# shenyunhang/PPS

Hardware: NVIDIA B200
Metric: qxg_pairs_per_sec_distance_plus_rank (higher is better)
Workload: dtype f16x3-split fp32 (two scaled fp16 planes, fp32 accumulate)

## Files before the change

pps_b200/build.py:

```python
from __future__ import annotations

import os
import shutil
import subprocess

HERE = os.path.dirname(os.path.abspath(__file__))
CSRC = os.path.join(HERE, "csrc")
OUT_DIR = os.path.join(HERE, "_C")
LIB_PATH = os.path.join(OUT_DIR, "libpps_b200.so")
SOURCES = ["pps_pool.cu", "split_prep.cu", "dist_gemm.cu", "pairs.cu", "rank.cu", "triplet.cu", "rerank.cu", "c_api.cu", "pass.cu", "index.cu"]
HEADERS = [os.path.join(CSRC, "common.cuh"), os.path.join(CSRC, "ctx.cuh"), os.path.join(CSRC, "dist_tiles.cuh"), os.path.join(os.path.dirname(HERE), "include", "pps_b200.h")]

NVCC_FLAGS = [
    "-gencode", "arch=compute_100a,code=sm_100a",
    "-O3", "-lineinfo", "-std=c++17",
    "-Xcompiler", "-fPIC",
]
OBJ_DIR = os.path.join(OUT_DIR, "obj")


def nvcc_path():
    for cand in (os.environ.get("NVCC"), shutil.which("nvcc"), "/usr/local/cuda/bin/nvcc"):
        if cand and os.path.exists(cand):
            return cand
    return None


def is_stale() -> bool:
    if not os.path.exists(LIB_PATH):
        return True
    t = os.path.getmtime(LIB_PATH)
    deps = [os.path.join(CSRC, s) for s in SOURCES] + HEADERS
    return any(os.path.getmtime(d) > t for d in deps if os.path.exists(d))


def _compile_one(nvcc, src, obj, verbose):
    cmd = [nvcc] + NVCC_FLAGS + (["-Xptxas", "-v"] if verbose else []) + ["-c", "-o", obj, src]
    proc = subprocess.run(cmd, cwd=CSRC, stdout=subprocess.PIPE, stderr=subprocess.STDOUT, text=True)
    return src, proc.returncode, proc.stdout


def build(force: bool = False, verbose: bool = False) -> str:
    if not force and not is_stale():
        return LIB_PATH
    nvcc = nvcc_path()
    if nvcc is None:
        raise RuntimeError("nvcc not found: cannot build libpps_b200.so (set NVCC or install the CUDA toolkit)")
    os.makedirs(OBJ_DIR, exist_ok=True)
    hdr_t = max(os.path.getmtime(h) for h in HEADERS if os.path.exists(h))
    jobs, objs = [], []
    for src in SOURCES:
        obj = os.path.join(OBJ_DIR, os.path.splitext(src)[0] + ".o")
        objs.append(obj)
        src_t = max(os.path.getmtime(os.path.join(CSRC, src)), hdr_t)
        if force or not os.path.exists(obj) or os.path.getmtime(obj) < src_t:
            jobs.append((src, obj))
    log = []
    if jobs:
        from concurrent.futures import ThreadPoolExecutor
        with ThreadPoolExecutor(max_workers=min(len(jobs), os.cpu_count() or 1)) as pool:
            for src, rc, out in pool.map(lambda j: _compile_one(nvcc, j[0], j[1], verbose), jobs):
                log.append("== %s ==\n%s" % (src, out))
                if rc != 0:
                    raise RuntimeError("nvcc failed on %s (%d):\n%s" % (src, rc, out))
    tmp = LIB_PATH + ".tmp.%d" % os.getpid()
    cmd = [nvcc, "-gencode", "arch=compute_100a,code=sm_100a", "-shared", "-o", tmp] + objs
    proc = subprocess.run(cmd, cwd=CSRC, stdout=subprocess.PIPE, stderr=subprocess.STDOUT, text=True)
    if proc.returncode != 0:
        if os.path.exists(tmp):
            os.remove(tmp)
        raise RuntimeError("nvcc link failed (%d):\n%s" % (proc.returncode, proc.stdout))
    os.replace(tmp, LIB_PATH)
    if verbose:
        print("\n".join(log))
    return LIB_PATH


TEST_HOOKS_PATH = os.path.join(OUT_DIR, "libpps_b200_testhooks.so")


def build_test_hooks(force: bool = False) -> str:
    src = os.path.join(CSRC, "test_hooks.cu")
    deps = [src] + [h for h in HEADERS if os.path.exists(h)]
    if (not force and os.path.exists(TEST_HOOKS_PATH)
            and all(os.path.getmtime(d) <= os.path.getmtime(TEST_HOOKS_PATH) for d in deps)):
        return TEST_HOOKS_PATH
    nvcc = nvcc_path()
    if nvcc is None:
        raise RuntimeError("nvcc not found: cannot build the test hooks")
    os.makedirs(OUT_DIR, exist_ok=True)
    tmp = TEST_HOOKS_PATH + ".tmp.%d" % os.getpid()
    proc = subprocess.run([nvcc] + NVCC_FLAGS + ["-shared", "-o", tmp, "test_hooks.cu"], cwd=CSRC, stdout=subprocess.PIPE,
                          stderr=subprocess.STDOUT, text=True)
    if proc.returncode != 0:
        raise RuntimeError("nvcc failed on test_hooks.cu:\n%s" % proc.stdout)
    os.replace(tmp, TEST_HOOKS_PATH)
    return TEST_HOOKS_PATH


if __name__ == "__main__":
    print(build(force=True, verbose=True))
```

pps_b200/csrc/c_api.cu:

```cuda
#include "common.cuh"

#include <algorithm>
#include <atomic>
#include <cstdio>
#include <cstring>
#include <new>
#include <numeric>
#include <string>
#include <vector>

namespace pps {

static std::atomic<unsigned long long> g_launches{0};
static thread_local std::string g_cuda_err;

void note_launch() { g_launches.fetch_add(1, std::memory_order_relaxed); }

int cuda_fail(cudaError_t e, const char* what) {
  g_cuda_err = std::string(what ? what : "?") + ": " + cudaGetErrorName(e) + " (" + cudaGetErrorString(e) + ")";
  return PPS_ERR_CUDA;
}

int sm_count() {
  static thread_local int cached_dev = -1, cached = 148;
// ... 26 lines not shown

using namespace pps;

extern "C" int pps_abi_version(void) { return PPS_ABI_VERSION; }

extern "C" const char* pps_strerror(int code) {
  switch (code) {
    case PPS_OK: return "ok";
    case PPS_ERR_INVALID_ARG: return "invalid argument (null pointer, negative size or unknown enum)";
    case PPS_ERR_SHAPE: return "shape check failed";
    case PPS_ERR_ALIGN: return "pointer or leading dimension not aligned";
    case PPS_ERR_CUDA: return "CUDA call failed";
    case PPS_ERR_UNSUPPORTED: return "request not supported by this build";
    case PPS_ERR_WORKSPACE: return "workspace too small";
    case PPS_ERR_NO_VALID_QUERY: return "No valid query";
    case PPS_ERR_PASS_RESIZE: return "a speculative size bound of the pass was too small: repeat it with PPS_PASS_SIZING";
    case PPS_ERR_TOPK_OVERFLOW: return "top-k candidate buffer overflow: repeat the pass with PPS_PASS_NO_EPILOGUE_TOPK";
    default: return "unknown error code";
  }
}

extern "C" const char* pps_last_cuda_error(void) { return g_cuda_err.c_str(); }

extern "C" unsigned long long pps_kernel_launch_count(void) { return g_launches.load(std::memory_order_relaxed); }

extern "C" long long pps_pairs_count(const int64_t* query_ids, long long nq, const int64_t* gallery_ids,
                                     long long ng) {
  if (nq < 0 || ng < 0 || ng > 0x7fffffffLL) return PPS_ERR_INVALID_ARG;
  if (nq == 0 || ng == 0) return 0;
  if (!query_ids || !gallery_ids) return PPS_ERR_INVALID_ARG;
  std::vector<int64_t> sorted(gallery_ids, gallery_ids + ng);
  std::sort(sorted.begin(), sorted.end());
  long long total = 0;
  for (long long i = 0; i < nq; ++i) {
    auto r = std::equal_range(sorted.begin(), sorted.end(), query_ids[i]);
    total += (long long)(r.second - r.first);
  }
  return total;
}

extern "C" int pps_pairs_fill(const int64_t* query_ids, const int64_t* query_cams, long long nq,
                              const int64_t* gallery_ids, const int64_t* gallery_cams, long long ng,
                              int32_t* pair_off, int32_t* pair_q, int32_t* pair_g, uint8_t* pair_pos) {
  if (nq < 0 || ng < 0 || ng > 0x7fffffffLL || nq > 0x7fffffffLL) return PPS_ERR_INVALID_ARG;
  if (!pair_off) return PPS_ERR_INVALID_ARG;
  pair_off[0] = 0;
  if (nq == 0) return PPS_OK;
  if (!query_ids || !query_cams || (ng > 0 && (!gallery_ids || !gallery_cams))) return PPS_ERR_INVALID_ARG;
  IdIndex idx(gallery_ids, ng);
  long long e = 0;
  for (long long i = 0; i < nq; ++i) {
    size_t lo, hi;
    idx.range(query_ids[i], &lo, &hi);
    if (e + (long long)(hi - lo) > 0x7fffffffLL) return PPS_ERR_UNSUPPORTED;
    for (size_t s = lo; s < hi; ++s, ++e) {
      const int32_t g = idx.order[s];
      if (!pair_q || !pair_g || !pair_pos) return PPS_ERR_INVALID_ARG;
      pair_q[e] = (int32_t)i;
      pair_g[e] = g;
      pair_pos[e] = gallery_cams[g] != query_cams[i] ? 1 : 0;
    }
    pair_off[i + 1] = (int32_t)e;
  }
  return PPS_OK;
}

#include "ctx.cuh"

namespace {
inline void mark(pps_ctx* c, int i, cudaStream_t s) {
  if (c->timing && c->ev_phase[i]) cudaEventRecord(c->ev_phase[i], s);
}
}

extern "C" int pps_ctx_create(int device, pps_ctx** out) {
  if (!out) return PPS_ERR_INVALID_ARG;
  *out = nullptr;
  PPS_CUDA_TRY(cudaSetDevice(device));
  pps_ctx* c = new (std::nothrow) pps_ctx();
  if (!c) return PPS_ERR_INVALID_ARG;
  c->device = device;
  cudaError_t e = cudaStreamCreateWithFlags(&c->copy_s, cudaStreamNonBlocking);
  if (e == cudaSuccess) e = cudaStreamCreateWithFlags(&c->comp_s, cudaStreamNonBlocking);
  if (e == cudaSuccess) e = cudaStreamCreateWithFlags(&c->side_s, cudaStreamNonBlocking);
  if (e == cudaSuccess) e = cudaEventCreateWithFlags(&c->ev_in, cudaEventDisableTiming);
  if (e == cudaSuccess) e = cudaEventCreateWithFlags(&c->ev_pairs, cudaEventDisableTiming);
  for (int i = 0; i < kMaxSlabs && e == cudaSuccess; ++i) e = cudaEventCreateWithFlags(&c->ev_slab[i], cudaEventDisableTiming);
  if (e == cudaSuccess) e = cudaEventCreateWithFlags(&c->ev_totals, cudaEventDisableTiming);
  for (int i = 0; i <= PPS_N_PHASES && e == cudaSuccess; ++i) e = cudaEventCreate(&c->ev_phase[i]);
  if (e != cudaSuccess) {
    pps_ctx_destroy(c);
    return cuda_fail(e, "pps_ctx_create");
  }
  *out = c;
  return PPS_OK;
}

extern "C" int pps_ctx_destroy(pps_ctx* c) {
  if (!c) return PPS_OK;
  cudaSetDevice(c->device);
  if (c->comp_s) cudaStreamSynchronize(c->comp_s);
  if (c->copy_s) cudaStreamSynchronize(c->copy_s);
  if (c->side_s) cudaStreamSynchronize(c->side_s);
  GrowBuf* bufs[] = {&c->qf, &c->gf, &c->qs, &c->gs, &c->qn, &c->gn, &c->dist, &c->ids, &c->pair_ws, &c->pair_off,
                     &c->totals, &c->pair_q, &c->pair_pos, &c->xbuf, &c->counters, &c->ap,
                     &c->valid, &c->first, &c->topk, &c->tki, &c->tkd};
  for (GrowBuf* b : bufs) b->release();
  c->h_small.release();
  c->pass.release();
  for (int i = 0; i < kMaxSlabs; ++i) if (c->ev_slab[i]) cudaEventDestroy(c->ev_slab[i]);
  if (c->ev_totals) cudaEventDestroy(c->ev_totals);
  if (c->ev_in) cudaEventDestroy(c->ev_in);
  if (c->ev_pairs) cudaEventDestroy(c->ev_pairs);
  if (c->side_s) cudaStreamDestroy(c->side_s);
  for (int i = 0; i <= PPS_N_PHASES; ++i) if (c->ev_phase[i]) cudaEventDestroy(c->ev_phase[i]);
  if (c->copy_s) cudaStreamDestroy(c->copy_s);
  if (c->comp_s) cudaStreamDestroy(c->comp_s);
  delete c;
  return PPS_OK;
}

namespace {

int eval_shape(long long nq, long long ng, long long col0, int dim, int precision, int topk, EvalShape* e) {
  if (nq <= 0 || ng <= 0 || dim <= 0 || topk < 0 || topk > PPS_TOPK_MAX || col0 < 0) return PPS_ERR_INVALID_ARG;
  if (nq > 0x7fffffffLL || col0 + ng > 0x7fffffffLL) return PPS_ERR_UNSUPPORTED;
  switch (precision) {
    case PPS_PREC_BF16X1: e->planes = 1; break;
    case PPS_PREC_BF16X3: e->planes = 2; break;
    case PPS_PREC_BF16X6: e->planes = 3; break;
    case PPS_PREC_F16X3: e->planes = 2; break;
    default: return PPS_ERR_INVALID_ARG;
  }
  e->split_planes = precision == PPS_PREC_F16X3 ? (2 | PPS_SPLIT_F16_SCALED) : e->planes;
  e->nq = nq; e->ng = ng; e->col0 = col0; e->dim = dim; e->precision = precision; e->topk = topk;
  e->ldd = (ng + 3) & ~3LL;
  e->kpad = pps_kpad(dim);
  if ((double)nq * (double)e->ldd * 4.0 > 64.0 * (double)(1LL << 30)) return PPS_ERR_UNSUPPORTED;
  return PPS_OK;
}

int ensure_common(pps_ctx* c, const EvalShape& e) {
  PPS_TRY(c->qs.ensure((size_t)pps_split_bytes(e.nq, e.dim, e.planes)));
  PPS_TRY(c->gs.ensure((size_t)pps_split_bytes(e.ng, e.dim, e.planes)));
  PPS_TRY(c->qn.ensure((size_t)e.nq * 8));
  PPS_TRY(c->gn.ensure((size_t)e.ng * 8));
  PPS_TRY(c->dist.ensure((size_t)e.nq * e.ldd * 4));
  PPS_TRY(c->pair_ws.ensure((size_t)pps_pairs_workspace_bytes(e.nq, e.ng)));
  PPS_TRY(c->pair_off.ensure(((size_t)e.nq + 1) * 4));
  PPS_TRY(c->totals.ensure(16));
  PPS_TRY(c->ap.ensure((size_t)e.nq * 8));
  PPS_TRY(c->valid.ensure((size_t)e.nq));
  PPS_TRY(c->first.ensure((size_t)e.nq * 4));
  const size_t off_ap = 16, off_first = off_ap + (size_t)e.nq * 8, off_valid = off_first + (size_t)e.nq * 4;
  PPS_TRY(c->h_small.ensure(off_valid + (size_t)e.nq));
  unsigned char* base = c->h_small.as<unsigned char>();
  c->st.totals = reinterpret_cast<int32_t*>(base);
  c->st.ap = reinterpret_cast<double*>(base + off_ap);
  c->st.first = reinterpret_cast<int32_t*>(base + off_first);
  c->st.valid = base + off_valid;
  return PPS_OK;
}

int pairs_local_count(pps_ctx* c, cudaStream_t ready_on) {
  const EvalShape& e = c->cur;
  cudaStream_t ps = c->pair_stream(ready_on);
  if (ready_on != ps) {
// ... 126 lines not shown

extern "C" int pps_evaluate_host_ctx(pps_ctx* c, const float* q_feats, long long nq, const float* g_feats, long long ng,
                                     int dim, const int64_t* query_ids, const int64_t* query_cams,
                                     const int64_t* gallery_ids, const int64_t* gallery_cams, int precision,
                                     int cmc_topk, int topk, double* out_map, double* out_cmc, double* out_ap,
                                     uint8_t* out_valid, int32_t* out_first_rank, int32_t* out_topk_index,
                                     float* out_topk_dist) {
  if (!c || cmc_topk < 0) return PPS_ERR_INVALID_ARG;
  PPS_TRY(eval_shape(nq, ng, 0, dim, precision, topk, &c->cur));
  c->world = 1;
  c->ext_pair_s = nullptr;
  const EvalShape& e = c->cur;
  if (!q_feats || !g_feats || !query_ids || !query_cams || !gallery_ids || !gallery_cams) return PPS_ERR_INVALID_ARG;
  if (!out_map || (cmc_topk > 0 && !out_cmc)) return PPS_ERR_INVALID_ARG;
  PPS_CUDA_TRY(cudaSetDevice(c->device));
  cudaStream_t cs = c->comp_s, ps = c->copy_s, ss = c->side_s;
  const int planes = e.planes, kpad = e.kpad;
  const long long ldd = e.ldd;

  PPS_TRY(ensure_common(c, e));
  PPS_TRY(c->qf.ensure((size_t)nq * dim * 4));
  PPS_TRY(c->gf.ensure((size_t)ng * dim * 4));
  PPS_TRY(c->ids.ensure((size_t)(2 * nq + 2 * ng) * 8));
  int64_t* d_qid = c->ids.as<int64_t>();
  int64_t* d_qcam = d_qid + nq;
  int64_t* d_gid = d_qcam + nq;
  int64_t* d_gcam = d_gid + ng;
  c->d_qid = d_qid; c->d_qcam = d_qcam; c->d_gid = d_gid; c->d_gcam = d_gcam;

  PPS_CUDA_TRY(cudaMemcpyAsync(d_qid, query_ids, (size_t)nq * 8, cudaMemcpyHostToDevice, ss));
  PPS_CUDA_TRY(cudaMemcpyAsync(d_qcam, query_cams, (size_t)nq * 8, cudaMemcpyHostToDevice, ss));
  PPS_CUDA_TRY(cudaMemcpyAsync(d_gid, gallery_ids, (size_t)ng * 8, cudaMemcpyHostToDevice, ss));
  PPS_CUDA_TRY(cudaMemcpyAsync(d_gcam, gallery_cams, (size_t)ng * 8, cudaMemcpyHostToDevice, ss));
  PPS_TRY(pairs_local_count(c, ss));
  PPS_TRY(pairs_offsets(c, c->local_cnt, 0, ss));

  PPS_CUDA_TRY(cudaMemcpyAsync(c->qf.p, q_feats, (size_t)nq * dim * 4, cudaMemcpyHostToDevice, cs));
  PPS_TRY(pps_split_rows(c->qf.p, PPS_DTYPE_F32, nq, dim, dim, e.split_planes, c->qs.p, c->qn.as<float>(), cs));

  long long slab = ((ng + 7) / 8 + 255) & ~255LL;
  if (slab < 1024) slab = 1024;
  while ((ng + slab - 1) / slab > kMaxSlabs) slab *= 2;
  int si = 0;
  const size_t esz = 2;
  for (long long r0 = 0; r0 < ng; r0 += slab, ++si) {
    const long long nr = std::min(slab, ng - r0);
    PPS_CUDA_TRY(cudaMemcpyAsync(c->gf.as<float>() + r0 * dim, g_feats + r0 * dim, (size_t)nr * dim * 4,
                                 cudaMemcpyHostToDevice, ps));
    PPS_CUDA_TRY(cudaEventRecord(c->ev_slab[si], ps));
    PPS_CUDA_TRY(cudaStreamWaitEvent(cs, c->ev_slab[si], 0));
    PPS_TRY(pps_split_rows_slab(c->gf.p, PPS_DTYPE_F32, r0, nr, ng, dim, dim, e.split_planes, c->gs.p, c->gn.as<float>(), cs));
    PPS_TRY(pps_dist_tc(c->qs.p, c->qn.as<float>(), nq, planes, 0,
                        c->gs.as<unsigned char>() + (size_t)r0 * kpad * esz, c->gn.as<float>() + r0, nr, planes, ng, dim,
                        precision, 0, c->dist.as<float>() + r0, ldd, cs));
  }
  int rc = pairs_and_thresholds(c, cs);
  if (rc == PPS_OK) rc = count_local(c, cs);
  if (rc == PPS_OK)
    rc = finalize_and_fetch(c, cmc_topk, cs, out_map, out_cmc, out_ap, out_valid, out_first_rank, out_topk_index,
                            out_topk_dist);
  cudaStreamSynchronize(ps);
  return rc;
}

extern "C" int pps_rank_begin(pps_ctx* c, const float* d_q, long long nq, const float* d_g, long long ng_local, int dim,
                              const int64_t* d_qid, const int64_t* d_qcam, const int64_t* d_gid_local,
                              const int64_t* d_gcam_local, long long gallery_offset, int world, int precision, int topk,
                              void* stream, void* pair_stream, int32_t** d_local_cnt) {
  if (!c || world < 1) return PPS_ERR_INVALID_ARG;
  PPS_TRY(eval_shape(nq, ng_local, gallery_offset, dim, precision, topk, &c->cur));
  if (!d_q || !d_g || !d_qid || !d_qcam || !d_gid_local || !d_gcam_local) return PPS_ERR_INVALID_ARG;
  PPS_CUDA_TRY(cudaSetDevice(c->device));
  cudaStream_t cs = static_cast<cudaStream_t>(stream);
  c->d_qid = d_qid; c->d_qcam = d_qcam; c->d_gid = d_gid_local; c->d_gcam = d_gcam_local;
  c->d_q = d_q; c->d_g = d_g;
  c->world = world;
  c->ext_pair_s = static_cast<cudaStream_t>(pair_stream);
  PPS_TRY(ensure_common(c, c->cur));
  const EvalShape& e = c->cur;
  mark(c, 0, cs);
  PPS_TRY(pairs_local_count(c, cs));
  if (d_local_cnt) *d_local_cnt = c->local_cnt;
  mark(c, 1, cs);
  PPS_TRY(pps_split_rows(d_q, PPS_DTYPE_F32, e.nq, e.dim, e.dim, e.split_planes, c->qs.p, c->qn.as<float>(), cs));
  PPS_TRY(pps_split_rows(d_g, PPS_DTYPE_F32, e.ng, e.dim, e.dim, e.split_planes, c->gs.p, c->gn.as<float>(), cs));
  mark(c, 2, cs);
  PPS_TRY(pps_dist_tc(c->qs.p, c->qn.as<float>(), e.nq, e.planes, 0, c->gs.p, c->gn.as<float>(), e.ng, e.planes, 0,
                      e.dim, e.precision, world > 1 ? PPS_DIST_RESERVE_SM_PAIR : 0, c->dist.as<float>(), e.ldd, cs));
  mark(c, 3, cs);
  return PPS_OK;
}

extern "C" int pps_rank_thresholds(pps_ctx* c, const int32_t* d_cnt_all, int rank, void* stream, long long* n_pairs,
                                   int32_t** d_exchange, long long* n_words) {
  if (!c || c->cur.nq <= 0 || rank < 0 || rank >= c->world) return PPS_ERR_INVALID_ARG;
  cudaStream_t cs = static_cast<cudaStream_t>(stream);
  PPS_TRY(pairs_offsets(c, d_cnt_all ? d_cnt_all : c->local_cnt, rank, cs));
  PPS_TRY(pairs_and_thresholds(c, cs));
  mark(c, 4, cs);
  if (n_pairs) *n_pairs = c->n_pairs;
  if (d_exchange) *d_exchange = c->xbuf.as<int32_t>();
  if (n_words) *n_words = 3 * c->n_pairs;
  return PPS_OK;
}

extern "C" int pps_rank_count_local(pps_ctx* c, void* stream, uint32_t** d_counters, long long* n_counters) {
  if (!c || c->cur.nq <= 0) return PPS_ERR_INVALID_ARG;
  cudaStream_t cs = static_cast<cudaStream_t>(stream);
  PPS_TRY(count_local(c, cs));
  mark(c, 5, cs);
  if (d_counters) *d_counters = c->counters.as<uint32_t>();
  if (n_counters) *n_counters = c->cur.nq + c->n_pairs;
  return PPS_OK;
}

extern "C" int pps_rank_end(pps_ctx* c, int cmc_topk, void* stream, double* out_map, double* out_cmc, double* out_ap,
                            uint8_t* out_valid, int32_t* out_first_rank, int32_t* out_topk_index,
                            float* out_topk_dist) {
  if (!c || c->cur.nq <= 0 || cmc_topk < 0) return PPS_ERR_INVALID_ARG;
  const int rc = finalize_and_fetch(c, cmc_topk, static_cast<cudaStream_t>(stream), out_map, out_cmc, out_ap, out_valid,
                                    out_first_rank, out_topk_index, out_topk_dist);
  if (rc == PPS_OK || rc == PPS_ERR_NO_VALID_QUERY) collect_phase_times(c);
  return rc;
}

extern "C" int pps_evaluate_device_ctx(pps_ctx* c, const float* d_q, long long nq, const float* d_g, long long ng,
                                       int dim, const int64_t* d_qid, const int64_t* d_qcam, const int64_t* d_gid,
                                       const int64_t* d_gcam, int precision, int cmc_topk, int topk, void* stream,
                                       double* out_map, double* out_cmc, double* out_ap, uint8_t* out_valid,
                                       int32_t* out_first_rank, int32_t* out_topk_index, float* out_topk_dist) {
  if (!out_map || (cmc_topk > 0 && !out_cmc)) return PPS_ERR_INVALID_ARG;
  PPS_TRY(pps_rank_begin(c, d_q, nq, d_g, ng, dim, d_qid, d_qcam, d_gid, d_gcam, 0, 1, precision, topk, stream, nullptr,
                         nullptr));
  PPS_TRY(pps_rank_thresholds(c, nullptr, 0, stream, nullptr, nullptr, nullptr));
  PPS_TRY(pps_rank_count_local(c, stream, nullptr, nullptr));
  return pps_rank_end(c, cmc_topk, stream, out_map, out_cmc, out_ap, out_valid, out_first_rank, out_topk_index,
                      out_topk_dist);
}

extern "C" int pps_ctx_set_timing(pps_ctx* c, int enabled) {
  if (!c) return PPS_ERR_INVALID_ARG;
  c->timing = enabled != 0;
  return PPS_OK;
}

extern "C" int pps_ctx_phase_ms(const pps_ctx* c, float* out_ms) {
  if (!c || !out_ms) return PPS_ERR_INVALID_ARG;
  for (int i = 0; i < PPS_N_PHASES; ++i) out_ms[i] = c->phase_ms[i];
  return PPS_OK;
}

extern "C" int pps_evaluate_host(const float* q_feats, long long nq, const float* g_feats, long long ng, int dim,
                                 const int64_t* query_ids, const int64_t* query_cams, const int64_t* gallery_ids,
                                 const int64_t* gallery_cams, int precision, int cmc_topk, int topk, int device,
                                 double* out_map, double* out_cmc, double* out_ap, uint8_t* out_valid,
                                 int32_t* out_first_rank, int32_t* out_topk_index, float* out_topk_dist) {
  pps_ctx* c = nullptr;
  int rc = pps_ctx_create(device, &c);
  if (rc != PPS_OK) return rc;
  rc = pps_evaluate_host_ctx(c, q_feats, nq, g_feats, ng, dim, query_ids, query_cams, gallery_ids, gallery_cams,
                             precision, cmc_topk, topk, out_map, out_cmc, out_ap, out_valid, out_first_rank,
                             out_topk_index, out_topk_dist);
  pps_ctx_destroy(c);
  return rc;
}
```

pps_b200/csrc/common.cuh:

```cuda
#pragma once

#include <cuda.h>
#include <cuda_runtime.h>
#include <cuda_bf16.h>
#include <cuda_fp16.h>
#include <stdint.h>

#include "../../include/pps_b200.h"

namespace pps {

void note_launch();
int  cuda_fail(cudaError_t e, const char* what);

#define PPS_CUDA_TRY(expr)                                            \
  do {                                                                \
    cudaError_t _e = (expr);                                          \
    if (_e != cudaSuccess) return ::pps::cuda_fail(_e, #expr);        \
  } while (0)

#define PPS_LAUNCH_CHECK(name)                                        \
  do {                                                                \
    ::pps::note_launch();                                             \
    cudaError_t _e = cudaGetLastError();                              \
    if (_e != cudaSuccess) return ::pps::cuda_fail(_e, name);         \
  } while (0)

int sm_count();

#ifdef __CUDACC__

__device__ __forceinline__ uint32_t smem_u32(const void* p) {
  return static_cast<uint32_t>(__cvta_generic_to_shared(p));
}

__device__ __forceinline__ void mbar_init(uint64_t* bar, uint32_t count) {
  asm volatile("mbarrier.init.shared::cta.b64 [%0], %1;" ::"r"(smem_u32(bar)), "r"(count) : "memory");
}
__device__ __forceinline__ void fence_barrier_init() {
  asm volatile("fence.mbarrier_init.release.cluster;" ::: "memory");
}
__device__ __forceinline__ void fence_proxy_async() {
  asm volatile("fence.proxy.async.shared::cta;" ::: "memory");
}
__device__ __forceinline__ void mbar_expect_tx(uint64_t* bar, uint32_t bytes) {
  asm volatile("mbarrier.arrive.expect_tx.shared::cta.b64 _, [%0], %1;" ::"r"(smem_u32(bar)), "r"(bytes)
               : "memory");
}
__device__ __forceinline__ void mbar_arrive(uint64_t* bar) {
  asm volatile("mbarrier.arrive.shared::cta.b64 _, [%0];" ::"r"(smem_u32(bar)) : "memory");
}
__device__ __forceinline__ bool mbar_try_wait(uint64_t* bar, uint32_t parity) {
  uint32_t ok;
  asm volatile(
      "{\n\t"
      ".reg .pred p;\n\t"
      "mbarrier.try_wait.parity.shared::cta.b64 p, [%1], %2;\n\t"
      "selp.u32 %0, 1, 0, p;\n\t"
      "}\n"
      : "=r"(ok)
      : "r"(smem_u32(bar)), "r"(parity)
      : "memory");
  return ok != 0;
}
__device__ __forceinline__ void mbar_wait(uint64_t* bar, uint32_t parity) {
  while (!mbar_try_wait(bar, parity)) {
  }
}

__device__ __forceinline__ void bulk_load_1d(void* smem_dst, const void* gsrc, uint32_t bytes, uint64_t* bar) {
  asm volatile(
      "cp.async.bulk.shared::cluster.global.mbarrier::complete_tx::bytes [%0], [%1], %2, [%3];" ::"r"(
          smem_u32(smem_dst)),
      "l"(gsrc), "r"(bytes), "r"(smem_u32(bar))
      : "memory");
}

__device__ __forceinline__ void tma_load_3d(void* smem_dst, const CUtensorMap* tmap, uint64_t* bar, int c0, int c1,
                                            int c2) {
  asm volatile(
      "cp.async.bulk.tensor.3d.shared::cluster.global.tile.mbarrier::complete_tx::bytes [%0], [%1, {%3, %4, %5}], "
      "[%2];" ::"r"(smem_u32(smem_dst)),
      "l"(reinterpret_cast<uint64_t>(tmap)), "r"(smem_u32(bar)), "r"(c0), "r"(c1), "r"(c2)
      : "memory");
}
__device__ __forceinline__ void tma_store_2d(const CUtensorMap* tmap, const void* smem_src, int c0, int c1) {
  asm volatile("cp.async.bulk.tensor.2d.global.shared::cta.tile.bulk_group [%0, {%2, %3}], [%1];" ::"l"(
                   reinterpret_cast<uint64_t>(tmap)),
               "r"(smem_u32(smem_src)), "r"(c0), "r"(c1)
               : "memory");
}
__device__ __forceinline__ void bulk_commit_group() { asm volatile("cp.async.bulk.commit_group;" ::: "memory"); }
template <int N>
__device__ __forceinline__ void bulk_wait_group_read() {
  asm volatile("cp.async.bulk.wait_group.read %0;" ::"n"(N) : "memory");
}
__device__ __forceinline__ float lds_f32(uint32_t addr) {
  float v;
  asm volatile("ld.shared.f32 %0, [%1];" : "=f"(v) : "r"(addr));
  return v;
}
__device__ __forceinline__ void red_shared_add_u32(uint32_t addr, uint32_t v) {
  asm volatile("red.shared.add.u32 [%0], %1;" ::"r"(addr), "r"(v) : "memory");
}
__device__ __forceinline__ uint32_t ld_volatile_u32(const uint32_t* p) {
  uint32_t v;
  asm volatile("ld.volatile.global.u32 %0, [%1];" : "=r"(v) : "l"(p) : "memory");
  return v;
}
__device__ __forceinline__ void st_volatile_u32(uint32_t* p, uint32_t v) {
  asm volatile("st.volatile.global.u32 [%0], %1;" ::"l"(p), "r"(v) : "memory");
// ... 148 lines not shown
```

pps_b200/csrc/ctx.cuh:

```cuda
#pragma once

#include "common.cuh"

#include <algorithm>
#include <cstring>
#include <new>
#include <vector>

namespace pps {

struct GrowBuf {
  void* p = nullptr;
  size_t cap = 0;
  int ensure(size_t bytes) {
    if (bytes <= cap) return PPS_OK;
    if (p) { cudaFree(p); p = nullptr; cap = 0; }
    const size_t want = bytes + bytes / 8 + 256;
    cudaError_t e = cudaMalloc(&p, want);
    if (e != cudaSuccess) { p = nullptr; return ::pps::cuda_fail(e, "cudaMalloc"); }
    cap = want;
    return PPS_OK;
  }
  void release() { if (p) cudaFree(p); p = nullptr; cap = 0; }
  template <class T> T* as() const { return static_cast<T*>(p); }
};

struct PinBuf {
  void* p = nullptr;
  size_t cap = 0;
  int ensure(size_t bytes) {
    if (bytes <= cap) return PPS_OK;
    if (p) { cudaFreeHost(p); p = nullptr; cap = 0; }
    cudaError_t e = cudaMallocHost(&p, bytes + 256);
    if (e != cudaSuccess) { p = nullptr; return ::pps::cuda_fail(e, "cudaMallocHost"); }
    cap = bytes + 256;
    return PPS_OK;
  }
  void release() { if (p) cudaFreeHost(p); p = nullptr; cap = 0; }
  template <class T> T* as() const { return static_cast<T*>(p); }
};

constexpr int kMaxSlabs = 64;

#define PPS_TRY(expr) do { int _rc = (expr); if (_rc != PPS_OK) return _rc; } while (0)

struct EvalShape {
  long long nq, ng , col0 , ldd;
  int dim, kpad, planes, precision, topk;
  int split_planes;
};
struct Staging {
  int32_t* totals; double* ap; int32_t* first; uint8_t* valid;
};

int pairs_count_device_ex(const int64_t* query_ids, long long nq, const int64_t* gallery_ids, long long ng_cap, void* workspace,
                          int32_t* pair_off, int32_t* totals, void* stream, const int32_t* ng_dev);
int pairs_fill_device_ex(const int64_t* query_ids, const int64_t* query_cams, long long nq, const int64_t* gallery_ids,
                         const int64_t* gallery_cams, long long ng_cap, const void* workspace, int32_t* pair_q, int32_t* pair_g,
                         uint8_t* pair_pos, float* zero_f32, uint32_t* zero_u32, uint32_t* zero_per_query, long long capacity,
                         void* stream, const int32_t* ng_dev);
int pairs_remap_ex(int32_t* pair_g, long long n_cap, const int32_t* cand_rows, long long offset, void* stream,
                   const int32_t* n_dev);
int pairs_compact_rows_ex(const int64_t* query_ids, long long nq, const int32_t* pair_off, const int32_t* pair_q,
                          const int32_t* pair_g, long long n_pairs, long long row_lo, long long row_hi, void* workspace,
                          int32_t* gp_rows, int32_t* pair_col, int32_t* n_rows, void* stream, const int32_t* n_pairs_dev,
                          long long rows_cap);
int rank_gather_ex(const float* dist, long long ldd, long long nq, long long ncols, long long col0, const int32_t* pair_q,
                   const int32_t* pair_g, long long n_pairs, float* pair_d, void* stream, const int32_t* n_dev);

constexpr int kPassMaxBlocks = 4096;
constexpr int kPassTimedLaunches = 256;
struct PassState {
  bool active = false;
  long long nq = 0, ngl = 0, ng_global = 0, offset = 0, chunk = 0, ldd = 0, n_pairs = 0, n_cand = 0, n_rows = 0;
  int dim = 0, kpad = 0, dtype = 0, planes = 0, split_planes = 0, precision = 0, topk = 0, world = 1, rank = 0, flags = 0;
  int max_pairs = 0, n_blocks = 0, tk_cap = 2048;
  bool prefilter = false, g_inplace = false, epi_topk = false;
  bool fused = false;
  int p_cap = 0;
  const void *d_q = nullptr, *d_g = nullptr;
  const void *h_q = nullptr, *h_g = nullptr;
  bool g_from_host = false;
  const int64_t *d_qid = nullptr, *d_qcam = nullptr, *d_gid = nullptr, *d_gcam = nullptr;
  long long blk_row0[kPassMaxBlocks], blk_rows[kPassMaxBlocks];
  size_t packed_bytes = 0;
  size_t res_bytes = 0, res_first_off = 0, res_valid_off = 0, res_flags_off = 0;
  GrowBuf qs, qn, gs, gn, dist, tdist, ts, tn, pair_ws, pair_off, totals, pair_q, pair_g, pair_pos, pair_d, packed, pf_ws,
      cand_rows, cand_gid, cand_gcam, gp_rows, pair_col, gp_ws, tk_bound, tk_cnt, tk_cand, small, ap, valid, first, tki, tkd,
      thr_tab, tpair_tab, cnt_tab, dstar, gstar;
  cudaEvent_t ev_a = nullptr, ev_rows = nullptr;
  cudaEvent_t ev_t[kPassTimedLaunches][2] = {};
  int n_timed = 0, timed_kind[kPassTimedLaunches] = {};
  float host_wait_ms[4] = {};
  struct Hints { bool valid = false; long long nq = 0, ng_global = 0, ngl = 0, offset = 0, mbb = 0; int dim = 0, dtype = 0, topk = 0,
                 world = 0, precision = 0; long long n_cand = 0, n_pairs = 0, n_rows = 0; int max_pairs = 0; } hints;
  bool speculative = false;
  long long cap_cand = 0, cap_rows = 0;
  void release() {
    GrowBuf* bufs[] = {&qs, &qn, &gs, &gn, &dist, &tdist, &ts, &tn, &pair_ws, &pair_off, &totals, &pair_q, &pair_g, &pair_pos,
                       &pair_d, &packed, &pf_ws, &cand_rows, &cand_gid, &cand_gcam, &gp_rows, &pair_col, &gp_ws, &tk_bound,
                       &tk_cnt, &tk_cand, &small, &ap, &valid, &first, &tki, &tkd, &thr_tab, &tpair_tab, &cnt_tab, &dstar, &gstar};
    for (GrowBuf* b : bufs) b->release();
    if (ev_a) cudaEventDestroy(ev_a);
    if (ev_rows) cudaEventDestroy(ev_rows);
    ev_a = ev_rows = nullptr;
    for (auto& e : ev_t) for (auto& x : e) { if (x) cudaEventDestroy(x); x = nullptr; }
  }
  unsigned long long* keys() const { return packed.as<unsigned long long>(); }
  uint32_t* cnt_first() const { return reinterpret_cast<uint32_t*>(packed.as<unsigned char>() + (size_t)nq * topk * 8); }
  uint32_t* cnt_le() const { return cnt_first() + nq; }
  uint32_t* flags_dev() const { return cnt_le() + n_pairs; }
  size_t counter_words() const { return (size_t)nq + (size_t)n_pairs + 2; }
};

}

struct pps_ctx {
  int device = 0;
  pps::PassState pass;
  cudaStream_t copy_s = nullptr, comp_s = nullptr, side_s = nullptr;
  cudaEvent_t ev_slab[pps::kMaxSlabs] = {};
  cudaEvent_t ev_totals = nullptr, ev_in = nullptr, ev_pairs = nullptr;
  pps::GrowBuf qf, gf, qs, gs, qn, gn, dist, ids, pair_ws, pair_off, totals, pair_q, pair_pos, xbuf, counters,
      ap, valid, first, topk, tki, tkd;
  pps::PinBuf h_small;
  pps::EvalShape cur = {};
  pps::Staging st = {};
  const int64_t *d_qid = nullptr, *d_qcam = nullptr, *d_gid = nullptr, *d_gcam = nullptr;
  const float *d_q = nullptr, *d_g = nullptr;
  long long n_pairs = 0;
  int max_pairs = 0;
  int world = 1;
  int32_t* local_cnt = nullptr;
  float* pair_d() const { return xbuf.as<float>(); }
  int32_t* pair_g() const { return xbuf.as<int32_t>() + n_pairs; }
  int32_t* pair_pos32() const { return xbuf.as<int32_t>() + 2 * n_pairs; }
  cudaStream_t ext_pair_s = nullptr;
  cudaStream_t pair_stream(cudaStream_t cs) const { return ext_pair_s ? ext_pair_s : (world == 1 ? side_s : cs); }
  bool timing = false;
  cudaEvent_t ev_phase[PPS_N_PHASES + 1] = {};
  float phase_ms[PPS_N_PHASES] = {};
};
```

pps_b200/csrc/pairs.cu:

```cuda
#include "common.cuh"

namespace pps {

constexpr int kPairQPerWarp = 4;
constexpr int kPairWarps = 8;
constexpr int kPairQPerCta = kPairQPerWarp * kPairWarps;

template <bool FILL>
__global__ void __launch_bounds__(32 * kPairWarps)
pairs_sweep_kernel(const int64_t* __restrict__ qid, const int64_t* __restrict__ qcam, int nq,
                   const int64_t* __restrict__ gid, const int64_t* __restrict__ gcam, long long ng, long long seg,
                   int nseg, int32_t* __restrict__ seg_cnt ,
                   const int32_t* __restrict__ my_base ,
                   long long g_offset , int32_t* __restrict__ pair_q,
                   int32_t* __restrict__ pair_g, uint8_t* __restrict__ pair_pos, int32_t* __restrict__ pair_pos32,
                   float* __restrict__ zero_f32, uint32_t* __restrict__ zero_u32,
                   uint32_t* __restrict__ zero_per_query, long long capacity,
                   const int32_t* __restrict__ ng_dev ) {
  if (ng_dev) ng = min(ng, (long long)*ng_dev);
  const int lane = threadIdx.x & 31, warp = threadIdx.x >> 5;
  const int q0 = blockIdx.x * kPairQPerCta + warp * kPairQPerWarp;
  const int s = blockIdx.y;
  if (q0 >= nq) return;
  int64_t ids[kPairQPerWarp], cams[kPairQPerWarp];
  int acc[kPairQPerWarp];
  bool live[kPairQPerWarp];
#pragma unroll
  for (int u = 0; u < kPairQPerWarp; ++u) {
    live[u] = q0 + u < nq;
    ids[u] = live[u] ? qid[q0 + u] : 0;
    cams[u] = (FILL && live[u]) ? qcam[q0 + u] : 0;
    acc[u] = 0;
    if (FILL && live[u]) {
      int part = 0;
      for (int sp = lane; sp < s; sp += 32) part += seg_cnt[(long long)(q0 + u) * nseg + sp];
#pragma unroll
      for (int o = 16; o > 0; o >>= 1) part += __shfl_xor_sync(0xffffffffu, part, o);
      acc[u] = my_base[q0 + u] + part;
      if (zero_per_query && s == 0 && lane == 0) zero_per_query[q0 + u] = 0u;
    }
  }
  const long long g_begin = (long long)s * seg;
  const long long g_end = min(ng, g_begin + seg);
  const unsigned lt = (1u << lane) - 1u;
  constexpr int kB = 8;
  for (long long g0 = g_begin; g0 < g_end; g0 += 32 * kB) {
    int64_t v[kB];
#pragma unroll
    for (int k = 0; k < kB; ++k) {
      const long long g = g0 + k * 32 + lane;
      v[k] = g < g_end ? gid[g] : 0;
    }
#pragma unroll
    for (int k = 0; k < kB; ++k) {
      const long long g = g0 + k * 32 + lane;
      const bool in = g < g_end;
      const uint32_t vlo = (uint32_t)v[k];
      bool maybe = false;
#pragma unroll
      for (int u = 0; u < kPairQPerWarp; ++u) maybe |= (vlo == (uint32_t)ids[u]);
      if (!__any_sync(0xffffffffu, maybe && in)) continue;
#pragma unroll
      for (int u = 0; u < kPairQPerWarp; ++u) {
        const bool hit = in && live[u] && v[k] == ids[u];
        const unsigned b = __ballot_sync(0xffffffffu, hit);
        if (FILL) {
          if (hit) {
            const long long slot = (long long)acc[u] + __popc(b & lt);
            if (slot < capacity) {
              pair_q[slot] = q0 + u;
              pair_g[slot] = (int32_t)(g + g_offset);
              const int pos = gcam[g] != cams[u] ? 1 : 0;
              if (pair_pos) pair_pos[slot] = (uint8_t)pos;
              if (pair_pos32) pair_pos32[slot] = pos;
              if (zero_f32) zero_f32[slot] = 0.f;
              if (zero_u32) zero_u32[slot] = 0u;
            }
          }
        }
        acc[u] += __popc(b);
      }
    }
  }
  if (!FILL && lane == 0) {
#pragma unroll
    for (int u = 0; u < kPairQPerWarp; ++u)
      if (live[u]) seg_cnt[(long long)(q0 + u) * nseg + s] = acc[u];
  }
}

__global__ void pairs_rowsum_kernel(const int32_t* __restrict__ seg_cnt, int nq, int nseg, int32_t* __restrict__ local_cnt) {
  const int q = blockIdx.x * blockDim.x + threadIdx.x;
  if (q >= nq) return;
  const int32_t* row = seg_cnt + (long long)q * nseg;
  int sum = 0;
  for (int sgi = 0; sgi < nseg; ++sgi) sum += row[sgi];
  local_cnt[q] = sum;
}

__global__ void __launch_bounds__(1024) pairs_offsets_kernel(const int32_t* __restrict__ cnt_all, int world, int rank,
                                                             int nq, int32_t* __restrict__ pair_off,
                                                             int32_t* __restrict__ my_base, int32_t* __restrict__ totals) {
  __shared__ int warp_sum[32];
  __shared__ int carry_s;
  __shared__ int max_s;
  const int tid = threadIdx.x, lane = tid & 31, warp = tid >> 5;
  if (tid == 0) { carry_s = 0; max_s = 0; }
  __syncthreads();
  int mx = 0;
  for (int base = 0; base < nq; base += 1024) {
    const int q = base + tid;
    int sum = 0, before = 0;
    if (q < nq) {
      for (int r = 0; r < world; ++r) {
        const int v = cnt_all[(long long)r * nq + q];
        sum += v;
        before += r < rank ? v : 0;
      }
    }
    mx = max(mx, sum);
    int incl = sum;
#pragma unroll
    for (int o = 1; o < 32; o <<= 1) {
      const int t = __shfl_up_sync(0xffffffffu, incl, o);
      if (lane >= o) incl += t;
    }
    if (lane == 31) warp_sum[warp] = incl;
    __syncthreads();
    if (warp == 0) {
      int w = warp_sum[lane];
#pragma unroll
      for (int o = 1; o < 32; o <<= 1) {
        const int t = __shfl_up_sync(0xffffffffu, w, o);
        if (lane >= o) w += t;
      }
      warp_sum[lane] = w;
    }
    __syncthreads();
    const int carry = carry_s;
    if (q < nq) {
      const int off = carry + (warp ? warp_sum[warp - 1] : 0) + incl - sum;
      pair_off[q] = off;
      my_base[q] = off + before;
    }
    __syncthreads();
    if (tid == 1023) carry_s = carry + warp_sum[31];
    __syncthreads();
  }
#pragma unroll
  for (int o = 16; o > 0; o >>= 1) mx = max(mx, __shfl_xor_sync(0xffffffffu, mx, o));
  if (lane == 0) atomicMax(&max_s, mx);
  __syncthreads();
  if (tid == 0) { pair_off[nq] = carry_s; totals[0] = carry_s; totals[1] = max_s; }
}

__global__ void pairs_unpack_pos_kernel(const int32_t* __restrict__ pos32, long long n, uint8_t* __restrict__ pos8) {
  const long long i = (long long)blockIdx.x * blockDim.x + threadIdx.x;
  if (i < n) pos8[i] = (uint8_t)(pos32[i] != 0);
}

static void pair_segments(long long ng, long long* seg, int* nseg) {
  long long s = 1024;
  while ((ng + s - 1) / s > 512) s *= 2;
  *seg = s;
  *nseg = (int)((ng + s - 1) / s);
  if (*nseg < 1) *nseg = 1;
}

__global__ void compact_hash_insert_kernel(int nq, const int32_t* __restrict__ pair_off, const int32_t* __restrict__ pair_g,
                                           int32_t* __restrict__ keys, int32_t* __restrict__ vals, uint32_t mask) {
  const int q = blockIdx.x * blockDim.x + threadIdx.x;
  if (q >= nq) return;
  const int e0 = pair_off[q];
  if (pair_off[q + 1] == e0) return;
  const int32_t g0 = pair_g[e0];
  uint32_t s = ((uint32_t)g0 * 0x9E3779B1u) & mask;
  while (true) {
    const int32_t old = atomicCAS(&keys[s], -1, g0);
    if (old == -1 || old == g0) { atomicMin(&vals[s], q); return; }
    s = (s + 1) & mask;
  }
}

__global__ void compact_rep_kernel(const int64_t* __restrict__ qid, int nq, const int32_t* __restrict__ pair_off,
                                   const int32_t* __restrict__ pair_g, int row_lo, int row_hi,
                                   const int32_t* __restrict__ keys, const int32_t* __restrict__ vals, uint32_t mask,
                                   int32_t* __restrict__ rep, int32_t* __restrict__ lo_out, int32_t* __restrict__ cnt) {
  const int q = blockIdx.x * blockDim.x + threadIdx.x;
  if (q >= nq) return;
  int r = q;
  if (pair_off[q + 1] > pair_off[q]) {
    const int32_t g0 = pair_g[pair_off[q]];
    uint32_t s = ((uint32_t)g0 * 0x9E3779B1u) & mask;
    while (keys[s] != g0) s = (s + 1) & mask;
    r = vals[s];
  }
  rep[q] = r;
  (void)qid;
  const int e0 = pair_off[q], e1 = pair_off[q + 1];
  int a = e0, b = e1;
  while (a < b) { const int m = (a + b) >> 1; if (pair_g[m] < row_lo) a = m + 1; else b = m; }
  const int lo = a;
  b = e1;
  while (a < b) { const int m = (a + b) >> 1; if (pair_g[m] < row_hi) a = m + 1; else b = m; }
  lo_out[q] = lo - e0;
  cnt[q] = a - lo;
}

__global__ void __launch_bounds__(1024) compact_scan_kernel(const int32_t* __restrict__ rep, const int32_t* __restrict__ cnt,
                                                            int nq, int32_t* __restrict__ gp_off,
                                                            int32_t* __restrict__ n_rows) {
  __shared__ int warp_sum[32];
  __shared__ int carry_s;
  const int tid = threadIdx.x, lane = tid & 31, warp = tid >> 5;
  if (tid == 0) carry_s = 0;
  __syncthreads();
  for (int base = 0; base < nq; base += 1024) {
    const int q = base + tid;
    const int v = (q < nq && rep[q] == q) ? cnt[q] : 0;
    int incl = v;
#pragma unroll
    for (int o = 1; o < 32; o <<= 1) {
      const int t = __shfl_up_sync(0xffffffffu, incl, o);
      if (lane >= o) incl += t;
    }
    if (lane == 31) warp_sum[warp] = incl;
    __syncthreads();
    if (warp == 0) {
      int w = warp_sum[lane];
#pragma unroll
      for (int o = 1; o < 32; o <<= 1) {
        const int t = __shfl_up_sync(0xffffffffu, w, o);
        if (lane >= o) w += t;
      }
      warp_sum[lane] = w;
    }
// ... 115 lines not shown
  __shared__ int carry_s;
  const int tid = threadIdx.x, lane = tid & 31, warp = tid >> 5;
  if (tid == 0) carry_s = 0;
  __syncthreads();
  for (int base = 0; base < n; base += 1024) {
    const int i = base + tid;
    const int v = i < n ? cnt[i] : 0;
    int incl = v;
#pragma unroll
    for (int o = 1; o < 32; o <<= 1) {
      const int t = __shfl_up_sync(0xffffffffu, incl, o);
      if (lane >= o) incl += t;
    }
    if (lane == 31) warp_sum[warp] = incl;
    __syncthreads();
    if (warp == 0) {
      int w = warp_sum[lane];
#pragma unroll
      for (int o = 1; o < 32; o <<= 1) {
        const int t = __shfl_up_sync(0xffffffffu, w, o);
        if (lane >= o) w += t;
      }
      warp_sum[lane] = w;
    }
    __syncthreads();
    const int carry = carry_s;
    if (i < n) cnt[i] = carry + (warp ? warp_sum[warp - 1] : 0) + incl - v;
    __syncthreads();
    if (tid == 1023) carry_s = carry + warp_sum[31];
    __syncthreads();
  }
  if (tid == 0) *n_out = carry_s;
}

__global__ void pairs_remap_kernel(int32_t* __restrict__ pair_g, long long n, const int32_t* __restrict__ cand_rows,
                                   long long offset, const int32_t* __restrict__ n_dev) {
  if (n_dev) n = min(n, (long long)*n_dev);
  const long long i = (long long)blockIdx.x * blockDim.x + threadIdx.x;
  if (i < n) pair_g[i] = (int32_t)(cand_rows[pair_g[i]] + offset);
}

__global__ void compact_pad_kernel(int32_t* __restrict__ gp_rows, const int32_t* __restrict__ n_rows, long long cap, int32_t pad) {
  const long long i = (long long)blockIdx.x * blockDim.x + threadIdx.x;
  if (i < cap && i >= (long long)*n_rows) gp_rows[i] = pad;
}

}

using namespace pps;

static long long ws_ints(long long nq, long long ng, int* nseg_out) {
  long long seg; int nseg;
  pair_segments(ng, &seg, &nseg);
  if (nseg_out) *nseg_out = nseg;
  return (nq > 0 ? nq : 1) * ((long long)nseg + 2);
}

extern "C" long long pps_pairs_workspace_bytes(long long nq, long long ng) {
  if (nq < 0 || ng < 0) return PPS_ERR_INVALID_ARG;
  return ws_ints(nq, ng, nullptr) * 4;
}

namespace pps {
int pairs_local_count_ex(const int64_t* query_ids, long long nq, const int64_t* gallery_ids, long long ng, void* workspace,
                         int32_t** local_cnt, void* stream, const int32_t* ng_dev) {
  if (nq < 0 || ng < 0 || nq > 0x7fffffffLL || ng > 0x7fffffffLL) return PPS_ERR_INVALID_ARG;
  if (!workspace) return PPS_ERR_INVALID_ARG;
  if (nq > 0 && ng > 0 && (!query_ids || !gallery_ids)) return PPS_ERR_INVALID_ARG;
  cudaStream_t st = static_cast<cudaStream_t>(stream);
  long long seg; int nseg;
  pair_segments(ng, &seg, &nseg);
  int32_t* seg_cnt = static_cast<int32_t*>(workspace);
  int32_t* lc = seg_cnt + (nq > 0 ? nq : 1) * (long long)nseg;
  if (local_cnt) *local_cnt = lc;
  if ((long long)nq * nseg > 0x7fffffffLL) return PPS_ERR_UNSUPPORTED;
  if (nq == 0) return PPS_OK;
  if (ng == 0) {
    PPS_CUDA_TRY(cudaMemsetAsync(seg_cnt, 0, (size_t)nq * (nseg + 1) * 4, st));
    return PPS_OK;
  }
  const dim3 grid((unsigned)((nq + kPairQPerCta - 1) / kPairQPerCta), (unsigned)nseg);
  pairs_sweep_kernel<false><<<grid, 32 * kPairWarps, 0, st>>>(query_ids, nullptr, (int)nq, gallery_ids, nullptr, ng, seg,
                                                              nseg, seg_cnt, nullptr, 0, nullptr, nullptr, nullptr,
                                                              nullptr, nullptr, nullptr, nullptr, 0, ng_dev);
  PPS_LAUNCH_CHECK("pairs_sweep_kernel<count>");
  pairs_rowsum_kernel<<<(unsigned)((nq + 255) / 256), 256, 0, st>>>(seg_cnt, (int)nq, nseg, lc);
  PPS_LAUNCH_CHECK("pairs_rowsum_kernel");
  return PPS_OK;
}
}

extern "C" int pps_pairs_local_count(const int64_t* query_ids, long long nq, const int64_t* gallery_ids, long long ng,
                                     void* workspace, int32_t** local_cnt, void* stream) {
  return pairs_local_count_ex(query_ids, nq, gallery_ids, ng, workspace, local_cnt, stream, nullptr);
}

extern "C" int pps_pairs_offsets(const int32_t* cnt_all, int world, int rank, long long nq, long long ng_local,
                                 void* workspace, int32_t* pair_off, int32_t* totals, void* stream) {
  if (nq < 0 || world < 1 || rank < 0 || rank >= world || nq > 0x7fffffffLL) return PPS_ERR_INVALID_ARG;
  if (!cnt_all || !workspace || !pair_off || !totals) return PPS_ERR_INVALID_ARG;
  int nseg;
  ws_ints(nq, ng_local, &nseg);
  int32_t* my_base = static_cast<int32_t*>(workspace) + (nq > 0 ? nq : 1) * ((long long)nseg + 1);
  pairs_offsets_kernel<<<1, 1024, 0, static_cast<cudaStream_t>(stream)>>>(cnt_all, world, rank, (int)nq, pair_off, my_base,
                                                                          totals);
  PPS_LAUNCH_CHECK("pairs_offsets_kernel");
  return PPS_OK;
}

namespace pps {
int pairs_fill_local_ex(const int64_t* query_ids, const int64_t* query_cams, long long nq, const int64_t* gallery_ids,
                        const int64_t* gallery_cams, long long ng, long long gallery_offset, const void* workspace,
                        int32_t* pair_q, int32_t* pair_g, uint8_t* pair_pos, int32_t* pair_pos32, float* zero_f32,
                        uint32_t* zero_u32, uint32_t* zero_per_query, long long capacity, void* stream, const int32_t* ng_dev) {
  if (nq < 0 || ng < 0 || nq > 0x7fffffffLL || ng > 0x7fffffffLL || capacity < 0 || gallery_offset < 0 ||
      gallery_offset + ng > 0x7fffffffLL)
    return PPS_ERR_INVALID_ARG;
  if (nq == 0) return PPS_OK;
  cudaStream_t st = static_cast<cudaStream_t>(stream);
  if (ng == 0 || capacity == 0) {
    if (zero_per_query) PPS_CUDA_TRY(cudaMemsetAsync(zero_per_query, 0, (size_t)nq * 4, st));
    return PPS_OK;
  }
  if (!query_ids || !query_cams || !gallery_ids || !gallery_cams || !workspace || !pair_q || !pair_g ||
      (!pair_pos && !pair_pos32))
    return PPS_ERR_INVALID_ARG;
  long long seg; int nseg;
  pair_segments(ng, &seg, &nseg);
  int32_t* seg_cnt = const_cast<int32_t*>(static_cast<const int32_t*>(workspace));
  const int32_t* my_base = seg_cnt + nq * ((long long)nseg + 1);
  const dim3 grid((unsigned)((nq + kPairQPerCta - 1) / kPairQPerCta), (unsigned)nseg);
  pairs_sweep_kernel<true><<<grid, 32 * kPairWarps, 0, st>>>(query_ids, query_cams, (int)nq, gallery_ids, gallery_cams, ng,
                                                             seg, nseg, seg_cnt, my_base, gallery_offset, pair_q, pair_g,
                                                             pair_pos, pair_pos32, zero_f32, zero_u32, zero_per_query,
                                                             capacity, ng_dev);
  PPS_LAUNCH_CHECK("pairs_sweep_kernel<fill>");
  return PPS_OK;
}

int pairs_remap_ex(int32_t* pair_g, long long n_cap, const int32_t* cand_rows, long long offset, void* stream,
                   const int32_t* n_dev) {
  if (n_cap <= 0) return PPS_OK;
  pairs_remap_kernel<<<(unsigned)((n_cap + 255) / 256), 256, 0, static_cast<cudaStream_t>(stream)>>>(pair_g, n_cap, cand_rows,
                                                                                                     offset, n_dev);
  PPS_LAUNCH_CHECK("pairs_remap_kernel");
  return PPS_OK;
}
}

extern "C" int pps_pairs_fill_local(const int64_t* query_ids, const int64_t* query_cams, long long nq,
                                    const int64_t* gallery_ids, const int64_t* gallery_cams, long long ng,
                                    long long gallery_offset, const void* workspace, int32_t* pair_q, int32_t* pair_g,
                                    uint8_t* pair_pos, int32_t* pair_pos32, float* zero_f32, uint32_t* zero_u32,
                                    uint32_t* zero_per_query, long long capacity, void* stream) {
  return pairs_fill_local_ex(query_ids, query_cams, nq, gallery_ids, gallery_cams, ng, gallery_offset, workspace, pair_q, pair_g,
                             pair_pos, pair_pos32, zero_f32, zero_u32, zero_per_query, capacity, stream, nullptr);
}

extern "C" int pps_pairs_unpack_pos(const int32_t* pair_pos32, long long n_pairs, uint8_t* pair_pos, void* stream) {
  if (n_pairs < 0) return PPS_ERR_INVALID_ARG;
  if (n_pairs == 0) return PPS_OK;
  if (!pair_pos32 || !pair_pos) return PPS_ERR_INVALID_ARG;
  pairs_unpack_pos_kernel<<<(unsigned)((n_pairs + 255) / 256), 256, 0, static_cast<cudaStream_t>(stream)>>>(
      pair_pos32, n_pairs, pair_pos);
  PPS_LAUNCH_CHECK("pairs_unpack_pos_kernel");
  return PPS_OK;
}

namespace pps {
int pairs_count_device_ex(const int64_t* query_ids, long long nq, const int64_t* gallery_ids, long long ng_cap, void* workspace,
                          int32_t* pair_off, int32_t* totals, void* stream, const int32_t* ng_dev) {
  if (!pair_off || !totals) return PPS_ERR_INVALID_ARG;
  int32_t* lc = nullptr;
  int rc = pairs_local_count_ex(query_ids, nq, gallery_ids, ng_cap, workspace, &lc, stream, ng_dev);
  if (rc != PPS_OK) return rc;
  return pps_pairs_offsets(lc, 1, 0, nq, ng_cap, workspace, pair_off, totals, stream);
}
int pairs_fill_device_ex(const int64_t* query_ids, const int64_t* query_cams, long long nq, const int64_t* gallery_ids,
                         const int64_t* gallery_cams, long long ng_cap, const void* workspace, int32_t* pair_q, int32_t* pair_g,
                         uint8_t* pair_pos, float* zero_f32, uint32_t* zero_u32, uint32_t* zero_per_query, long long capacity,
                         void* stream, const int32_t* ng_dev) {
  return pairs_fill_local_ex(query_ids, query_cams, nq, gallery_ids, gallery_cams, ng_cap, 0, workspace, pair_q, pair_g,
                             pair_pos, nullptr, zero_f32, zero_u32, zero_per_query, capacity, stream, ng_dev);
}
}

extern "C" int pps_pairs_count_device(const int64_t* query_ids, long long nq, const int64_t* gallery_ids, long long ng,
                                      void* workspace, int32_t* pair_off, int32_t* totals, void* stream) {
  if (!pair_off || !totals) return PPS_ERR_INVALID_ARG;
  int32_t* lc = nullptr;
  int rc = pps_pairs_local_count(query_ids, nq, gallery_ids, ng, workspace, &lc, stream);
  if (rc != PPS_OK) return rc;
  return pps_pairs_offsets(lc, 1, 0, nq, ng, workspace, pair_off, totals, stream);
}

extern "C" int pps_pairs_fill_device(const int64_t* query_ids, const int64_t* query_cams, long long nq,
                                     const int64_t* gallery_ids, const int64_t* gallery_cams, long long ng,
                                     const void* workspace, int32_t* pair_q, int32_t* pair_g, uint8_t* pair_pos,
                                     float* zero_f32, uint32_t* zero_u32, uint32_t* zero_per_query, long long capacity,
                                     void* stream) {
  return pps_pairs_fill_local(query_ids, query_cams, nq, gallery_ids, gallery_cams, ng, 0, workspace, pair_q, pair_g,
                              pair_pos, nullptr, zero_f32, zero_u32, zero_per_query, capacity, stream);
}

static uint32_t compact_slots(long long nq) {
  uint32_t n = 64;
  while ((long long)n < 2 * nq) n <<= 1;
  return n;
}

extern "C" long long pps_pairs_compact_workspace_bytes(long long nq) {
  if (nq < 0 || nq > 0x3fffffffLL) return PPS_ERR_INVALID_ARG;
  return (4 * (nq > 0 ? nq : 1) + 4) * 4 + (long long)compact_slots(nq) * 8;
}

namespace pps {
int pairs_compact_rows_ex(const int64_t* query_ids, long long nq, const int32_t* pair_off, const int32_t* pair_q,
                          const int32_t* pair_g, long long n_pairs, long long row_lo, long long row_hi, void* workspace,
                          int32_t* gp_rows, int32_t* pair_col, int32_t* n_rows, void* stream, const int32_t* n_pairs_dev,
                          long long rows_cap ) {
  if (nq < 0 || n_pairs < 0 || row_lo < 0 || row_hi < row_lo || nq > 0x7fffffffLL || row_hi > 0x7fffffffLL)
    return PPS_ERR_INVALID_ARG;
  if (!n_rows) return PPS_ERR_INVALID_ARG;
  cudaStream_t st = static_cast<cudaStream_t>(stream);
  if (nq == 0 || n_pairs == 0) {
    PPS_CUDA_TRY(cudaMemsetAsync(n_rows, 0, 4, st));
    return PPS_OK;
  }
  if (!query_ids || !pair_off || !pair_q || !pair_g || !workspace || !gp_rows || !pair_col) return PPS_ERR_INVALID_ARG;
  int32_t* rep = static_cast<int32_t*>(workspace);
  int32_t* lo = rep + nq;
  int32_t* cnt = lo + nq;
  int32_t* gp_off = cnt + nq;
  const uint32_t slots = compact_slots(nq);
  int32_t* keys = gp_off + nq + 4;
  int32_t* vals = keys + slots;
  PPS_CUDA_TRY(cudaMemsetAsync(keys, 0xFF, (size_t)slots * 4, st));
  PPS_CUDA_TRY(cudaMemsetAsync(vals, 0x7F, (size_t)slots * 4, st));
  compact_hash_insert_kernel<<<(unsigned)((nq + 127) / 128), 128, 0, st>>>((int)nq, pair_off, pair_g, keys, vals, slots - 1);
  PPS_LAUNCH_CHECK("compact_hash_insert_kernel");
  compact_rep_kernel<<<(unsigned)((nq + 127) / 128), 128, 0, st>>>(query_ids, (int)nq, pair_off, pair_g, (int)row_lo,
                                                                   (int)row_hi, keys, vals, slots - 1, rep, lo, cnt);
  PPS_LAUNCH_CHECK("compact_rep_kernel");
  compact_scan_kernel<<<1, 1024, 0, st>>>(rep, cnt, (int)nq, gp_off, n_rows);
  PPS_LAUNCH_CHECK("compact_scan_kernel");
  compact_fill_kernel<<<(unsigned)((n_pairs + 255) / 256), 256, 0, st>>>(pair_off, pair_q, pair_g, n_pairs, rep, lo, cnt,
                                                                         gp_off, gp_rows, pair_col, n_pairs_dev);
  PPS_LAUNCH_CHECK("compact_fill_kernel");
  if (rows_cap > 0) {
    compact_pad_kernel<<<(unsigned)((rows_cap + 255) / 256), 256, 0, st>>>(gp_rows, n_rows, rows_cap, (int32_t)row_lo);
    PPS_LAUNCH_CHECK("compact_pad_kernel");
  }
  return PPS_OK;
}
}

extern "C" int pps_pairs_compact_rows(const int64_t* query_ids, long long nq, const int32_t* pair_off,
                                      const int32_t* pair_q, const int32_t* pair_g, long long n_pairs, long long row_lo,
                                      long long row_hi, void* workspace, int32_t* gp_rows, int32_t* pair_col,
// ... 60 lines not shown
```

pps_b200/csrc/pass.cu:

```cuda
#include "ctx.cuh"

#include <chrono>
#include <cmath>

namespace pps {

constexpr int kTkCap = 2048;
constexpr long long kPrefilterMinRows = 32768;
constexpr long long kThreshCols = 32768;

__global__ void pass_reduce_counters_kernel(const unsigned char* __restrict__ gathered, size_t stride_bytes, size_t off_bytes,
                                            int world, long long n_words, uint32_t* __restrict__ out) {
  const long long i = (long long)blockIdx.x * blockDim.x + threadIdx.x;
  if (i >= n_words) return;
  uint32_t s = 0;
  for (int r = 0; r < world; ++r) s += reinterpret_cast<const uint32_t*>(gathered + (size_t)r * stride_bytes + off_bytes)[i];
  out[i] = s;
}

__global__ void __launch_bounds__(256) pass_merge_keys_kernel(const unsigned char* __restrict__ gathered, size_t stride_bytes,
                                                              int world, int k, int n_pow2,
                                                              unsigned long long* __restrict__ out) {
  extern __shared__ unsigned long long keys_s[];
  const int q = blockIdx.x, tid = threadIdx.x;
  const int n = world * k;
  for (int i = tid; i < n_pow2; i += 256) {
    unsigned long long v = ~0ull;
    if (i < n) {
      const int r = i / k, j = i - r * k;
      v = reinterpret_cast<const unsigned long long*>(gathered + (size_t)r * stride_bytes)[(long long)q * k + j];
    }
    keys_s[i] = v;
  }
  __syncthreads();
  for (int kk = 2; kk <= n_pow2; kk <<= 1) {
    for (int j = kk >> 1; j > 0; j >>= 1) {
      for (int i = tid; i < n_pow2; i += 256) {
        const int ixj = i ^ j;
        if (ixj > i) {
          const unsigned long long x = keys_s[i], y = keys_s[ixj];
          const bool up = (i & kk) == 0;
          if ((x > y) == up) { keys_s[i] = y; keys_s[ixj] = x; }
        }
      }
      __syncthreads();
    }
  }
  for (int i = tid; i < k; i += 256) out[(long long)q * k + i] = keys_s[i];
}

__global__ void pass_or_flag_kernel(const int32_t* __restrict__ src, uint32_t* __restrict__ dst) {
  if (threadIdx.x == 0 && blockIdx.x == 0 && *src) *dst = 1u;
}

__global__ void pass_copy_flags_kernel(const uint32_t* __restrict__ src, uint32_t* __restrict__ dst) {
  if (threadIdx.x < 2 && blockIdx.x == 0) dst[threadIdx.x] = src[threadIdx.x];
}

__global__ void pass_clamp_offsets_kernel(int32_t* __restrict__ pair_off, long long n, int32_t cap) {
  const long long i = (long long)blockIdx.x * blockDim.x + threadIdx.x;
  if (i < n && pair_off[i] > cap) pair_off[i] = cap;
}

__global__ void pass_check_bounds_kernel(const int32_t* __restrict__ tot, int32_t cap_pairs, int32_t cap_maxp, int32_t cap_cand,
                                         int32_t cap_rows, uint32_t* __restrict__ flag) {
  if (threadIdx.x == 0 && blockIdx.x == 0) {
    const bool bad = tot[0] > cap_pairs || tot[1] > cap_maxp || (cap_cand >= 0 && tot[2] > cap_cand) ||
                     (cap_rows >= 0 && tot[3] > cap_rows);
    if (bad) *flag = 1u;
  }
}

}

using namespace pps;

namespace {

int plan_blocks(PassState& p, bool short_first) {
  p.n_blocks = 0;
  const long long ngl = p.ngl, block_rows = p.chunk;
  if (ngl <= 0) return PPS_OK;
  long long first = std::min(block_rows, ngl);
  if (short_first && p.topk > 0) {
    long long want = (long long)(2.2 * p.topk * (double)std::min(block_rows, ngl) / kTkCap);
    want = std::max<long long>(16384, (want + 255) / 256 * 256);
    if (ngl >= 4 * want) first = std::min(first, want);
  }
  long long r0 = 0, rows = first;
  while (r0 < ngl) {
    if (p.n_blocks >= kPassMaxBlocks) return PPS_ERR_UNSUPPORTED;
    p.blk_row0[p.n_blocks] = r0;
    p.blk_rows[p.n_blocks] = rows;
    ++p.n_blocks;
    r0 += rows;
    rows = std::min(block_rows, ngl - r0);
  }
  return PPS_OK;
}

struct HostWait {
  pps_ctx* c; int slot; std::chrono::steady_clock::time_point t0;
  HostWait(pps_ctx* c_, int slot_) : c(c_), slot(slot_), t0(std::chrono::steady_clock::now()) {}
  ~HostWait() {
    if (c->timing) c->pass.host_wait_ms[slot] += std::chrono::duration<float, std::milli>(std::chrono::steady_clock::now() - t0).count();
  }
};

struct TimedLaunch {
  pps_ctx* c; cudaStream_t s; int slot;
  TimedLaunch(pps_ctx* c_, cudaStream_t s_, int kind) : c(c_), s(s_), slot(-1) {
    PassState& p = c->pass;
    if (!c->timing || p.n_timed >= kPassTimedLaunches) return;
    slot = p.n_timed++;
    p.timed_kind[slot] = kind;
    for (int i = 0; i < 2; ++i)
      if (!p.ev_t[slot][i]) cudaEventCreate(&p.ev_t[slot][i]);
    cudaEventRecord(p.ev_t[slot][0], s);
  }
  ~TimedLaunch() { if (slot >= 0) cudaEventRecord(c->pass.ev_t[slot][1], s); }
};

int split_block(pps_ctx* c, int blk, long long r0, long long rows, cudaStream_t cs, const void** planes_out) {
  PassState& p = c->pass;
  const size_t esz = p.dtype == PPS_DTYPE_F16 ? 2 : 4;
  const unsigned char* src = static_cast<const unsigned char*>(p.d_g) + (size_t)r0 * p.dim * esz;
  if (p.g_from_host && blk >= 0) PPS_CUDA_TRY(cudaStreamWaitEvent(cs, c->ev_slab[blk], 0));
  TimedLaunch t(c, cs, 1);
  if (p.g_inplace) {
    *planes_out = src;
    return pps_row_sqnorm(src, PPS_DTYPE_F16, rows, p.dim, p.dim, p.gn.as<float>(), cs);
  }
  *planes_out = p.gs.p;
  return pps_split_rows(src, p.dtype, rows, p.dim, p.dim, p.split_planes, p.gs.p, p.gn.as<float>(), cs);
}

int distance_block(pps_ctx* c, const void* g_planes, long long rows, long long col0, bool admit, cudaStream_t cs) {
  PassState& p = c->pass;
  TimedLaunch t(c, cs, 2);
  if (admit)
    return pps_dist_topk_tc(p.qs.p, p.qn.as<float>(), p.nq, p.planes, 0, g_planes, p.gn.as<float>(), rows, p.planes, 0, p.dim,
                            p.precision, 0, p.dist.as<float>(), p.ldd, col0, p.tk_bound.as<uint32_t>(),
                            p.tk_cnt.as<uint32_t>(), p.tk_cand.as<uint64_t>(), p.tk_cap, cs);
  return pps_dist_tc(p.qs.p, p.qn.as<float>(), p.nq, p.planes, 0, g_planes, p.gn.as<float>(), rows, p.planes, 0, p.dim,
// ... 32 lines not shown
  p.dtype = dtype; p.precision = precision; p.topk = topk; p.world = world; p.rank = rank; p.flags = flags;
  p.split_planes = precision == PPS_PREC_F16X3 ? (2 | PPS_SPLIT_F16_SCALED) : p.planes;
  p.d_q = d_q; p.d_g = d_g; p.d_qid = d_qid; p.d_qcam = d_qcam; p.d_gid = d_gid; p.d_gcam = d_gcam;
  p.g_inplace = dtype == PPS_DTYPE_F16 && (dim % 64) == 0 && (reinterpret_cast<uintptr_t>(d_g) & 15u) == 0;
  p.n_timed = 0;
  for (float& w : p.host_wait_ms) w = 0.f;
  p.tk_cap = (flags >> 8) & 0xffff;
  if (p.tk_cap <= 0 || p.tk_cap > kTkCap) p.tk_cap = kTkCap;
  if (!p.ev_a) PPS_CUDA_TRY(cudaEventCreateWithFlags(&p.ev_a, cudaEventDisableTiming));
  if (!p.ev_rows) PPS_CUDA_TRY(cudaEventCreateWithFlags(&p.ev_rows, cudaEventDisableTiming));

  long long chunk = std::max<long long>(256, std::min<long long>(std::max<long long>(ng_local, 1), max_block_bytes / (4 * nq)));
  if (chunk < ng_local) chunk = std::max<long long>(256, chunk / 256 * 256);
  p.chunk = chunk;
  p.ldd = (std::min(chunk, std::max<long long>(ng_local, 1)) + 3) / 4 * 4;
  const bool want_epi = topk > 0 && !(flags & PPS_PASS_NO_EPILOGUE_TOPK);
  PPS_TRY(plan_blocks(p, want_epi));
  p.epi_topk = want_epi && p.n_blocks > 1;
  if (p.n_blocks > 0) {
    long long mx = 0;
    for (int b = 0; b < p.n_blocks; ++b) mx = std::max(mx, p.blk_rows[b]);
    p.ldd = (mx + 3) / 4 * 4;
  }

  PPS_TRY(p.qs.ensure((size_t)pps_split_bytes(nq, dim, p.planes)));
  PPS_TRY(p.qn.ensure((size_t)nq * 8));
  if (!p.g_inplace) PPS_TRY(p.gs.ensure((size_t)pps_split_bytes(std::max<long long>(p.ldd, 1), dim, p.planes)));
  PPS_TRY(p.gn.ensure((size_t)std::max<long long>(p.ldd, 1) * 8));
  PPS_TRY(p.dist.ensure((size_t)nq * p.ldd * 4));
  PPS_TRY(p.pair_off.ensure(((size_t)nq + 1) * 4));
  PPS_TRY(p.totals.ensure(64));
  const size_t off_ap = 64, off_first = off_ap + (size_t)nq * 8, off_valid = off_first + (size_t)nq * 4;
  const size_t off_flags = (off_valid + (size_t)nq + 7) & ~(size_t)7;
  p.res_bytes = off_flags + 8 - off_ap;
  PPS_TRY(p.ap.ensure(p.res_bytes));
  PPS_TRY(c->h_small.ensure(off_flags + 8));
  unsigned char* hb = c->h_small.as<unsigned char>();
  c->st.totals = reinterpret_cast<int32_t*>(hb);
  c->st.ap = reinterpret_cast<double*>(hb + off_ap);
  c->st.first = reinterpret_cast<int32_t*>(hb + off_first);
  c->st.valid = hb + off_valid;
  p.res_first_off = off_first - off_ap; p.res_valid_off = off_valid - off_ap; p.res_flags_off = off_flags - off_ap;
  int32_t* h_tot = c->st.totals;

  PPS_CUDA_TRY(cudaEventRecord(c->ev_in, cs));
  PPS_CUDA_TRY(cudaStreamWaitEvent(ss, c->ev_in, 0));
  p.prefilter = ng_global >= kPrefilterMinRows;
  if (p.prefilter) {
    PPS_TRY(p.pf_ws.ensure((size_t)pps_pairs_prefilter_workspace_bytes(nq, ng_global)));
    PPS_TRY(p.cand_rows.ensure((size_t)ng_global * 4));
    PPS_TRY(p.cand_gid.ensure((size_t)ng_global * 8));
    PPS_TRY(p.cand_gcam.ensure((size_t)ng_global * 8));
    PPS_TRY(pps_pairs_prefilter(d_qid, nq, d_gid, d_gcam, ng_global, p.pf_ws.p, p.cand_rows.as<int32_t>(),
                                p.cand_gid.as<int64_t>(), p.cand_gcam.as<int64_t>(), p.totals.as<int32_t>() + 2, ss));
    PPS_CUDA_TRY(cudaMemcpyAsync(h_tot + 2, p.totals.as<int32_t>() + 2, 4, cudaMemcpyDeviceToHost, ss));
    PPS_CUDA_TRY(cudaEventRecord(p.ev_a, ss));
  }

  const size_t esz_in = dtype == PPS_DTYPE_F16 ? 2 : 4;
  const void* h_q = p.h_q;
  const void* h_g = p.h_g;
  p.h_q = p.h_g = nullptr;
  p.g_from_host = false;
  if (h_q) PPS_CUDA_TRY(cudaMemcpyAsync(const_cast<void*>(d_q), h_q, (size_t)nq * dim * esz_in, cudaMemcpyHostToDevice, cs));
  bool slabbed = false;
  if (h_g && ng_local > 0) {
    unsigned char* dg = static_cast<unsigned char*>(const_cast<void*>(d_g));
    const unsigned char* hg = static_cast<const unsigned char*>(h_g);
    PPS_CUDA_TRY(cudaStreamWaitEvent(c->copy_s, c->ev_in, 0));
    if (p.n_blocks == 1) {
      slabbed = true;
    } else if (p.n_blocks <= kMaxSlabs) {
      p.g_from_host = true;
      for (int b = 0; b < p.n_blocks; ++b) {
        const size_t off = (size_t)p.blk_row0[b] * dim * esz_in;
        PPS_CUDA_TRY(cudaMemcpyAsync(dg + off, hg + off, (size_t)p.blk_rows[b] * dim * esz_in, cudaMemcpyHostToDevice, c->copy_s));
        PPS_CUDA_TRY(cudaEventRecord(c->ev_slab[b], c->copy_s));
      }
    } else {
      PPS_CUDA_TRY(cudaMemcpyAsync(dg, hg, (size_t)ng_local * dim * esz_in, cudaMemcpyHostToDevice, cs));
    }
  }

  {
    TimedLaunch t(c, cs, 1);
    PPS_TRY(pps_split_rows(d_q, dtype, nq, dim, dim, p.split_planes, p.qs.p, p.qn.as<float>(), cs));
  }
  const void* gp0 = nullptr;
  long long slab = 0;
  if (slabbed) {
    unsigned char* dg = static_cast<unsigned char*>(const_cast<void*>(d_g));
    const unsigned char* hg = static_cast<const unsigned char*>(h_g);
    slab = ((ng_local + 7) / 8 + 255) & ~255LL;
    if (slab < 1024) slab = 1024;
    while ((ng_local + slab - 1) / slab > kMaxSlabs) slab *= 2;
    int si = 0;
    for (long long r0 = 0; r0 < ng_local; r0 += slab, ++si) {
      const long long nr = std::min(slab, ng_local - r0);
      const size_t off = (size_t)r0 * dim * esz_in;
      PPS_CUDA_TRY(cudaMemcpyAsync(dg + off, hg + off, (size_t)nr * dim * esz_in, cudaMemcpyHostToDevice, c->copy_s));
      PPS_CUDA_TRY(cudaEventRecord(c->ev_slab[si], c->copy_s));
    }
  } else if (p.n_blocks > 0) {
    PPS_TRY(split_block(c, 0, p.blk_row0[0], p.blk_rows[0], cs, &gp0));
  }

  PassState::Hints& hn = p.hints;
  p.speculative = !(flags & PPS_PASS_SIZING) && hn.valid && hn.nq == nq && hn.ng_global == ng_global && hn.ngl == ng_local &&
                  hn.offset == gallery_offset && hn.mbb == max_block_bytes && hn.dim == dim && hn.dtype == dtype &&
                  hn.topk == topk && hn.world == world && hn.precision == precision;
  const bool spec = p.speculative;
  int32_t* d_tot = p.totals.as<int32_t>();
  const int64_t* sweep_gid = d_gid;
  const int64_t* sweep_gcam = d_gcam;
  long long sweep_rows = ng_global;
  const int32_t* dn_cand = nullptr;
  if (p.prefilter) {
    if (spec) {
      p.cap_cand = std::min<long long>(ng_global, (hn.n_cand + 1023) / 1024 * 1024);
    } else {
      {
        HostWait hw(c, 0);
        PPS_CUDA_TRY(cudaEventSynchronize(p.ev_a));
      }
      p.n_cand = h_tot[2];
      p.cap_cand = p.n_cand;
    }
    sweep_gid = p.cand_gid.as<int64_t>(); sweep_gcam = p.cand_gcam.as<int64_t>(); sweep_rows = p.cap_cand;
    dn_cand = d_tot + 2;
  }
  PPS_TRY(p.pair_ws.ensure((size_t)std::max<long long>(pps_pairs_workspace_bytes(nq, sweep_rows), 16)));
  PPS_TRY(pairs_count_device_ex(d_qid, nq, sweep_gid, sweep_rows, p.pair_ws.p, p.pair_off.as<int32_t>(), d_tot, ss, dn_cand));
  if (spec) {
    p.n_pairs = hn.n_pairs > 0 ? (hn.n_pairs + hn.n_pairs / 8 + 1023) / 1024 * 1024 : 0;
    p.max_pairs = hn.max_pairs > 0 ? (hn.max_pairs + 8 + 15) / 16 * 16 : 0;
    pass_clamp_offsets_kernel<<<(unsigned)((nq + 1 + 255) / 256), 256, 0, ss>>>(p.pair_off.as<int32_t>(), nq + 1, (int32_t)p.n_pairs);
    PPS_LAUNCH_CHECK("pass_clamp_offsets_kernel");
  } else {
    PPS_CUDA_TRY(cudaMemcpyAsync(h_tot, d_tot, 8, cudaMemcpyDeviceToHost, ss));
    PPS_CUDA_TRY(cudaEventRecord(c->ev_totals, ss));
    {
      HostWait hw(c, 1);
      PPS_CUDA_TRY(cudaEventSynchronize(c->ev_totals));
    }
    p.n_pairs = h_tot[0];
    p.max_pairs = h_tot[1];
  }
  const int32_t* dn_pairs = spec ? d_tot : nullptr;
  const size_t np1 = (size_t)std::max<long long>(p.n_pairs, 1);
  {
    const int need = spec ? hn.max_pairs + 8 : p.max_pairs;
    p.fused = p.n_blocks > 1 && p.planes == 1 && p.n_pairs > 0 && need <= 64 && !(flags & PPS_PASS_NO_FUSED_COUNT) &&
              (topk == 0 || p.epi_topk);
    p.p_cap = std::max(8, (need + 7) / 8 * 8);
  }
  PPS_TRY(p.small.ensure(16));
  PPS_CUDA_TRY(cudaMemsetAsync(p.small.p, 0, 16, ss));
  PPS_TRY(p.pair_q.ensure(np1 * 4));
  PPS_TRY(p.pair_g.ensure(np1 * 4));
  PPS_TRY(p.pair_pos.ensure(np1));
  PPS_TRY(p.pair_d.ensure(np1 * 4));
  p.packed_bytes = ((size_t)nq * topk * 8 + p.counter_words() * 4 + 15) & ~(size_t)15;
  PPS_TRY(p.packed.ensure(p.packed_bytes));
  if (spec) {
    PPS_CUDA_TRY(cudaMemsetAsync(p.pair_d.p, 0, np1 * 4, ss));
    PPS_CUDA_TRY(cudaMemsetAsync(p.cnt_first(), 0, p.counter_words() * 4, ss));
    PPS_CUDA_TRY(cudaMemsetAsync(p.pair_q.p, 0xFF, np1 * 4, ss));
    PPS_CUDA_TRY(cudaMemsetAsync(p.pair_pos.p, 0, np1, ss));
    PPS_CUDA_TRY(cudaMemsetAsync(p.pair_g.p, 0, np1 * 4, ss));
  } else {
    PPS_CUDA_TRY(cudaMemsetAsync(p.flags_dev(), 0, 8, ss));
    if (p.n_pairs == 0) PPS_CUDA_TRY(cudaMemsetAsync(p.cnt_first(), 0, (size_t)nq * 4, ss));
  }
  PPS_TRY(pairs_fill_device_ex(d_qid, d_qcam, nq, sweep_gid, sweep_gcam, sweep_rows, p.pair_ws.p, p.pair_q.as<int32_t>(),
                               p.pair_g.as<int32_t>(), p.pair_pos.as<uint8_t>(), p.pair_d.as<float>(), p.cnt_le(),
                               p.cnt_first(), p.n_pairs, ss, dn_cand));
  if (p.prefilter && p.n_pairs > 0)
    PPS_TRY(pairs_remap_ex(p.pair_g.as<int32_t>(), p.n_pairs, p.cand_rows.as<int32_t>(), 0, ss, dn_pairs));
  if (topk > 0) {
    PPS_TRY(pps_topk_init(reinterpret_cast<uint64_t*>(p.keys()), nq, topk, ss));
    if (p.epi_topk) {
      PPS_TRY(p.tk_bound.ensure((size_t)nq * 4));
      PPS_TRY(p.tk_cnt.ensure((size_t)nq * 4));
      PPS_TRY(p.tk_cand.ensure((size_t)nq * p.tk_cap * 8));
    }
  }
  p.n_rows = 0;
  p.cap_rows = 0;
  PPS_CUDA_TRY(cudaMemsetAsync(d_tot + 3, 0, 4, ss));
  if (p.n_blocks > 1 && p.n_pairs > 0) {
    PPS_TRY(p.gp_ws.ensure((size_t)pps_pairs_compact_workspace_bytes(nq)));
    if (spec) p.cap_rows = hn.n_rows > 0 ? std::min<long long>((hn.n_rows + 255) / 256 * 256, std::max<long long>(p.ngl, 1)) : 0;
    PPS_TRY(p.gp_rows.ensure(std::max(np1, (size_t)p.cap_rows) * 4));
    PPS_TRY(p.pair_col.ensure(np1 * 4));
    PPS_TRY(pairs_compact_rows_ex(d_qid, nq, p.pair_off.as<int32_t>(), p.pair_q.as<int32_t>(), p.pair_g.as<int32_t>(),
                                  p.n_pairs, p.offset, p.offset + p.ngl, p.gp_ws.p, p.gp_rows.as<int32_t>(),
                                  p.pair_col.as<int32_t>(), d_tot + 3, ss, dn_pairs, spec ? p.cap_rows : 0));
    if (spec) {
      p.n_rows = p.cap_rows;
    } else {
      PPS_CUDA_TRY(cudaMemcpyAsync(h_tot + 3, d_tot + 3, 4, cudaMemcpyDeviceToHost, ss));
      PPS_CUDA_TRY(cudaEventRecord(p.ev_rows, ss));
      {
        HostWait hw(c, 2);
        PPS_CUDA_TRY(cudaEventSynchronize(p.ev_rows));
      }
      p.n_rows = h_tot[3];
    }
  }
  if (!spec) {
    hn.valid = true; hn.nq = nq; hn.ng_global = ng_global; hn.ngl = ng_local; hn.offset = gallery_offset; hn.mbb = max_block_bytes;
    hn.dim = dim; hn.dtype = dtype; hn.topk = topk; hn.world = world; hn.precision = precision;
    hn.n_cand = p.prefilter ? p.n_cand : 0; hn.n_pairs = p.n_pairs; hn.max_pairs = p.max_pairs; hn.n_rows = p.n_rows;
  }
  PPS_CUDA_TRY(cudaEventRecord(c->ev_pairs, ss));

  if (slabbed) {
    unsigned char* dg = static_cast<unsigned char*>(const_cast<void*>(d_g));
    int si = 0;
    for (long long r0 = 0; r0 < ng_local; r0 += slab, ++si) {
      const long long nr = std::min(slab, ng_local - r0);
      const size_t off = (size_t)r0 * dim * esz_in;
      PPS_CUDA_TRY(cudaStreamWaitEvent(cs, c->ev_slab[si], 0));
      const void* bp;
      {
        TimedLaunch t(c, cs, 1);
        if (p.g_inplace) {
          bp = dg + off;
          PPS_TRY(pps_row_sqnorm(dg + off, PPS_DTYPE_F16, nr, dim, dim, p.gn.as<float>() + r0, cs));
        } else {
          bp = p.gs.as<unsigned char>() + (size_t)r0 * p.kpad * 2;
          PPS_TRY(pps_split_rows_slab(dg, dtype, r0, nr, ng_local, dim, dim, p.split_planes, p.gs.p, p.gn.as<float>(), cs));
        }
      }
      TimedLaunch t(c, cs, 2);
      PPS_TRY(pps_dist_tc(p.qs.p, p.qn.as<float>(), nq, p.planes, 0, bp, p.gn.as<float>() + r0, nr, p.planes, ng_local, dim,
                          precision, world > 1 ? PPS_DIST_RESERVE_SM_PAIR : 0, p.dist.as<float>() + r0, p.ldd, cs));
    }
  } else if (p.n_blocks > 0) {
    PPS_TRY(distance_block(c, gp0, p.blk_rows[0], p.offset + p.blk_row0[0], false, cs));
  }
  PPS_CUDA_TRY(cudaStreamWaitEvent(cs, c->ev_pairs, 0));

  if (p.n_pairs > 0 && p.n_blocks == 1) {
    PPS_TRY(rank_gather_ex(p.dist.as<float>(), p.ldd, nq, p.blk_rows[0], p.offset, p.pair_q.as<int32_t>(),
                           p.pair_g.as<int32_t>(), p.n_pairs, p.pair_d.as<float>(), cs, dn_pairs));
  } else if (p.n_rows > 0) {
    if (p.g_from_host)
      PPS_CUDA_TRY(cudaStreamWaitEvent(cs, c->ev_slab[p.n_blocks - 1], 0));
    const long long tcols = std::min<long long>(p.n_rows, kThreshCols);
    const long long ldt = (tcols + 3) / 4 * 4;
    PPS_TRY(p.tdist.ensure((size_t)nq * ldt * 4));
    PPS_TRY(p.ts.ensure((size_t)pps_split_bytes(tcols, dim, p.planes)));
    PPS_TRY(p.tn.ensure((size_t)tcols * 8));
    for (long long c0 = 0; c0 < p.n_rows; c0 += tcols) {
      const long long rows = std::min(tcols, p.n_rows - c0);
      {
        TimedLaunch t(c, cs, 1);
        PPS_TRY(pps_split_rows_gather(d_g, dtype, p.gp_rows.as<int32_t>() + c0, p.offset, rows, dim, dim, p.split_planes,
                                      p.ts.p, p.tn.as<float>(), cs));
      }
      {
        TimedLaunch t(c, cs, 2);
        PPS_TRY(pps_dist_tc(p.qs.p, p.qn.as<float>(), nq, p.planes, 0, p.ts.p, p.tn.as<float>(), rows, p.planes, 0, dim,
                            precision, 0, p.tdist.as<float>(), ldt, cs));
      }
      PPS_TRY(rank_gather_ex(p.tdist.as<float>(), ldt, nq, rows, c0, p.pair_q.as<int32_t>(), p.pair_col.as<int32_t>(),
                             p.n_pairs, p.pair_d.as<float>(), cs, dn_pairs));
    }
  }
  p.active = true;
  if (d_x1) *d_x1 = p.pair_d.as<int32_t>();
  if (n_x1) *n_x1 = p.n_pairs;
  return PPS_OK;
}

extern "C" int pps_pass_count(pps_ctx* c, const void* d_gathered_x1, void* stream, void** d_x2, long long* x2_bytes) {
  if (!c || !c->pass.active) return PPS_ERR_INVALID_ARG;
  PassState& p = c->pass;
  if (p.world > 1 && p.n_pairs > 0 && !d_gathered_x1) return PPS_ERR_INVALID_ARG;
  cudaStream_t cs = static_cast<cudaStream_t>(stream);
  const bool have_pairs = p.n_pairs > 0;
  if (p.world > 1 && have_pairs) {
    pass_reduce_counters_kernel<<<(unsigned)((p.n_pairs + 255) / 256), 256, 0, cs>>>(
        static_cast<const unsigned char*>(d_gathered_x1), (size_t)p.n_pairs * 4, 0, p.world, p.n_pairs,
        p.pair_d.as<uint32_t>());
    PPS_LAUNCH_CHECK("pass_reduce_counters_kernel");
  }
  auto count_block = [&](long long rows, long long col0, bool with_topk) -> int {
    TimedLaunch t(c, cs, 4);
    if (with_topk)
      return pps_rank_sweep(p.dist.as<float>(), p.ldd, p.nq, rows, col0, p.pair_off.as<int32_t>(),
                            have_pairs ? p.pair_g.as<int32_t>() : nullptr, have_pairs ? p.pair_pos.as<uint8_t>() : nullptr,
                            have_pairs ? p.pair_d.as<float>() : nullptr, have_pairs ? p.max_pairs : 0,
                            have_pairs ? p.cnt_le() : nullptr, p.cnt_first(), reinterpret_cast<uint64_t*>(p.keys()), p.topk,
                            1, cs);
    if (!have_pairs) return PPS_OK;
    return pps_rank_count(p.dist.as<float>(), p.ldd, p.nq, rows, col0, p.pair_off.as<int32_t>(), p.pair_g.as<int32_t>(),
                          p.pair_pos.as<uint8_t>(), p.pair_d.as<float>(), p.max_pairs, p.cnt_le(), p.cnt_first(), cs);
  };
  if (p.fused) {
    const size_t elems = (size_t)pps_rank_tab_elems(p.nq, p.p_cap);
    PPS_TRY(p.thr_tab.ensure(elems * 4));
    PPS_TRY(p.tpair_tab.ensure(elems * 4));
    PPS_TRY(p.cnt_tab.ensure(elems * 4));
    PPS_TRY(p.dstar.ensure((size_t)p.nq * 4));
    PPS_TRY(p.gstar.ensure((size_t)p.nq * 4));
    TimedLaunch t(c, cs, 4);
    PPS_TRY(pps_rank_tab_prep(p.nq, p.pair_off.as<int32_t>(), p.pair_g.as<int32_t>(), p.pair_pos.as<uint8_t>(),
                              p.pair_d.as<float>(), p.p_cap, p.thr_tab.as<float>(), p.tpair_tab.as<int32_t>(),
                              p.cnt_tab.as<uint32_t>(), p.dstar.as<float>(), p.gstar.as<int32_t>(), p.small.as<int32_t>() + 1, cs));
  }
  for (int b = 0; b < p.n_blocks; ++b) {
    const long long r0 = p.blk_row0[b], rows = p.blk_rows[b], col0 = p.offset + r0;
    if (b == 0) {
      PPS_TRY(count_block(rows, col0, p.topk > 0));
      continue;
    }
    const void* gp = nullptr;
    PPS_TRY(split_block(c, b, r0, rows, cs, &gp));
    if (p.fused) {
      if (p.epi_topk && b == 1)
        PPS_TRY(pps_topk_bound(reinterpret_cast<const uint64_t*>(p.keys()), p.nq, p.topk, p.tk_bound.as<uint32_t>(),
                               p.tk_cnt.as<uint32_t>(), cs));
      {
        TimedLaunch t(c, cs, 2);
        PPS_TRY(pps_dist_rank_topk_tc(p.qs.p, p.qn.as<float>(), p.nq, p.planes, 0, gp, p.gn.as<float>(), rows, p.planes, 0,
                                      p.dim, p.precision, 0, col0, p.p_cap, p.thr_tab.as<float>(), p.cnt_tab.as<uint32_t>(),
                                      p.dstar.as<float>(), p.gstar.as<int32_t>(), p.cnt_first(),
                                      p.epi_topk ? p.tk_bound.as<uint32_t>() : nullptr,
                                      p.epi_topk ? p.tk_cnt.as<uint32_t>() : nullptr,
                                      p.epi_topk ? p.tk_cand.as<uint64_t>() : nullptr, p.tk_cap, cs));
      }
      if (p.epi_topk) {
        TimedLaunch t(c, cs, 4);
        PPS_TRY(pps_topk_merge(reinterpret_cast<uint64_t*>(p.keys()), p.nq, p.topk, p.tk_cand.as<uint64_t>(), p.tk_cap,
                               p.tk_cnt.as<uint32_t>(), p.tk_bound.as<uint32_t>(), p.pair_off.as<int32_t>(),
                               p.pair_g.as<int32_t>(), p.pair_pos.as<uint8_t>(), p.max_pairs, 1, p.small.as<int32_t>(), cs));
      }
    } else if (p.epi_topk) {
      if (b == 1)
        PPS_TRY(pps_topk_bound(reinterpret_cast<const uint64_t*>(p.keys()), p.nq, p.topk, p.tk_bound.as<uint32_t>(),
                               p.tk_cnt.as<uint32_t>(), cs));
      PPS_TRY(distance_block(c, gp, rows, col0, true, cs));
      PPS_TRY(count_block(rows, col0, false));
      TimedLaunch t(c, cs, 4);
      PPS_TRY(pps_topk_merge(reinterpret_cast<uint64_t*>(p.keys()), p.nq, p.topk, p.tk_cand.as<uint64_t>(), p.tk_cap,
                             p.tk_cnt.as<uint32_t>(), p.tk_bound.as<uint32_t>(), p.pair_off.as<int32_t>(),
                             have_pairs ? p.pair_g.as<int32_t>() : nullptr, have_pairs ? p.pair_pos.as<uint8_t>() : nullptr,
                             have_pairs ? p.max_pairs : 0, 1, p.small.as<int32_t>(), cs));
    } else {
      PPS_TRY(distance_block(c, gp, rows, col0, false, cs));
      PPS_TRY(count_block(rows, col0, p.topk > 0));
    }
  }
  if (p.fused) {
    TimedLaunch t(c, cs, 4);
    PPS_TRY(pps_rank_tab_finish(p.nq, p.p_cap, p.tpair_tab.as<int32_t>(), p.cnt_tab.as<uint32_t>(), p.cnt_le(), cs));
    pass_or_flag_kernel<<<1, 32, 0, cs>>>(p.small.as<int32_t>() + 1, p.flags_dev() + 1);
    PPS_LAUNCH_CHECK("pass_or_flag_kernel");
  }
  if (p.speculative) {
    pass_check_bounds_kernel<<<1, 32, 0, cs>>>(p.totals.as<int32_t>(), (int32_t)p.n_pairs, (int32_t)p.max_pairs,
                                               p.prefilter ? (int32_t)p.cap_cand : -1,
                                               p.n_blocks > 1 ? (int32_t)p.cap_rows : -1, p.flags_dev() + 1);
    PPS_LAUNCH_CHECK("pass_check_bounds_kernel");
  }
  if (p.epi_topk) {
    pass_or_flag_kernel<<<1, 32, 0, cs>>>(p.small.as<int32_t>(), p.flags_dev());
    PPS_LAUNCH_CHECK("pass_or_flag_kernel");
  }
  if (d_x2) *d_x2 = p.packed.p;
  if (x2_bytes) *x2_bytes = (long long)p.packed_bytes;
  return PPS_OK;
}

extern "C" int pps_pass_end(pps_ctx* c, const void* d_gathered, int cmc_topk, void* stream, double* out_map, double* out_cmc,
                            double* out_ap, uint8_t* out_valid, int32_t* out_first_rank, int32_t* out_topk_index,
                            float* out_topk_dist) {
  if (!c || !c->pass.active || cmc_topk < 0) return PPS_ERR_INVALID_ARG;
  PassState& p = c->pass;
  if (p.world > 1 && !d_gathered) return PPS_ERR_INVALID_ARG;
  cudaStream_t cs = static_cast<cudaStream_t>(stream);
  const long long nq = p.nq;
  const int topk = p.topk;
  if (p.world > 1) {
    const unsigned char* gth = static_cast<const unsigned char*>(d_gathered);
    const long long words = (long long)p.counter_words();
    pass_reduce_counters_kernel<<<(unsigned)((words + 255) / 256), 256, 0, cs>>>(gth, p.packed_bytes, (size_t)nq * topk * 8,
                                                                                p.world, words, p.cnt_first());
    PPS_LAUNCH_CHECK("pass_reduce_counters_kernel");
    if (topk > 0) {
      int n_pow2 = 2;
      while (n_pow2 < p.world * topk) n_pow2 <<= 1;
      pass_merge_keys_kernel<<<(unsigned)nq, 256, (size_t)n_pow2 * 8, cs>>>(gth, p.packed_bytes, p.world, topk, n_pow2, p.keys());
      PPS_LAUNCH_CHECK("pass_merge_keys_kernel");
    }
  }
  {
    TimedLaunch t(c, cs, 5);
    PPS_TRY(pps_rank_finalize(nq, p.pair_off.as<int32_t>(), p.pair_g.as<int32_t>(), p.pair_pos.as<uint8_t>(),
                              p.pair_d.as<float>(), p.cnt_le(), p.cnt_first(), p.ap.as<double>(),
                              p.ap.as<uint8_t>() + p.res_valid_off,
                              reinterpret_cast<int32_t*>(p.ap.as<unsigned char>() + p.res_first_off), nullptr, cs));
    pass_copy_flags_kernel<<<1, 32, 0, cs>>>(p.flags_dev(), reinterpret_cast<uint32_t*>(p.ap.as<unsigned char>() + p.res_flags_off));
    PPS_LAUNCH_CHECK("pass_copy_flags_kernel");
    if (topk > 0) {
      PPS_TRY(p.tki.ensure((size_t)nq * topk * 4));
      PPS_TRY(p.tkd.ensure((size_t)nq * topk * 4));
      PPS_TRY(pps_topk_unpack(reinterpret_cast<const uint64_t*>(p.keys()), nq, topk, p.tkd.as<float>(), p.tki.as<int32_t>(), cs));
    }
  }
  const Staging& st = c->st;
  PPS_CUDA_TRY(cudaMemcpyAsync(st.ap, p.ap.p, p.res_bytes, cudaMemcpyDeviceToHost, cs));
  if (topk > 0 && out_topk_index)
    PPS_CUDA_TRY(cudaMemcpyAsync(out_topk_index, p.tki.p, (size_t)nq * topk * 4, cudaMemcpyDeviceToHost, cs));
  if (topk > 0 && out_topk_dist)
    PPS_CUDA_TRY(cudaMemcpyAsync(out_topk_dist, p.tkd.p, (size_t)nq * topk * 4, cudaMemcpyDeviceToHost, cs));
  {
    HostWait hw(c, 3);
    PPS_CUDA_TRY(cudaStreamSynchronize(cs));
  }
  p.active = false;
  if (c->timing) {
    for (int i = 0; i < PPS_N_PHASES; ++i) c->phase_ms[i] = 0.f;
    for (int i = 0; i < p.n_timed; ++i) {
      float ms = 0.f;
      if (cudaEventElapsedTime(&ms, p.ev_t[i][0], p.ev_t[i][1]) == cudaSuccess) c->phase_ms[p.timed_kind[i]] += ms;
    }
    c->phase_ms[0] = p.host_wait_ms[0] + p.host_wait_ms[1] + p.host_wait_ms[2];
    c->phase_ms[6] = p.host_wait_ms[3];
  }
  const uint32_t* h_flags = reinterpret_cast<const uint32_t*>(reinterpret_cast<const unsigned char*>(st.ap) + p.res_flags_off);
  if (h_flags[1] != 0) {
    p.hints.valid = false;
    return PPS_ERR_PASS_RESIZE;
  }
  if (h_flags[0] != 0) return PPS_ERR_TOPK_OVERFLOW;
  double ap_sum = 0.0;
  long long n_valid = 0;
  std::vector<double> hist((size_t)std::max(cmc_topk, 1), 0.0);
  for (long long i = 0; i < nq; ++i) {
    if (!st.valid[i]) continue;
    ++n_valid;
    ap_sum += st.ap[i];
    if (st.first[i] >= 0 && st.first[i] < cmc_topk) hist[(size_t)st.first[i]] += 1.0;
  }
  if (out_ap) std::memcpy(out_ap, st.ap, (size_t)nq * 8);
  if (out_valid) std::memcpy(out_valid, st.valid, (size_t)nq);
  if (out_first_rank) std::memcpy(out_first_rank, st.first, (size_t)nq * 4);
  if (n_valid == 0) return PPS_ERR_NO_VALID_QUERY;
  if (out_map) *out_map = ap_sum / (double)n_valid;
  double run = 0.0;
  for (int k = 0; k < cmc_topk && out_cmc; ++k) {
    run += hist[(size_t)k];
    out_cmc[k] = run / (double)n_valid;
  }
  return PPS_OK;
}

extern "C" long long pps_pass_stat(const pps_ctx* c, int which) {
  if (!c) return -1;
  const PassState& p = c->pass;
  switch (which) {
    case 0: return p.n_blocks;
    case 1: return p.fused ? 1 : 0;
    case 2: return p.speculative ? 1 : 0;
    case 3: return p.fused ? p.p_cap : 0;
    case 4: return p.epi_topk ? 1 : 0;
    default: return -1;
  }
}

extern "C" int pps_pass_set_host_input(pps_ctx* c, const void* h_q, const void* h_g) {
  if (!c) return PPS_ERR_INVALID_ARG;
  c->pass.h_q = h_q;
  c->pass.h_g = h_g;
  return PPS_OK;
}
```

pps_b200/csrc/rank.cu:

```cuda
#include "common.cuh"

#include <cfloat>

namespace pps {

constexpr int kCntThreads = 128;
constexpr int kNB = 1024;

__device__ __forceinline__ int fkey(float x) {
  const int k = __float_as_int(x);
  return k ^ ((k >> 31) & 0x7fffffff);
}

constexpr int kTopkThreads = 256;
constexpr int kCand = 2048;

__device__ __noinline__ void bitonic_sort_smem(unsigned long long* a, int n , int tid, int nthreads) {
  for (int k = 2; k <= n; k <<= 1) {
    for (int j = k >> 1; j > 0; j >>= 1) {
      for (int i = tid; i < n; i += nthreads) {
        const int ixj = i ^ j;
        if (ixj > i) {
          const unsigned long long x = a[i], y = a[ixj];
          const bool up = (i & k) == 0;
// ... 255 lines not shown
    if (!count_on) return;
  } else if (vec) {
    const long long c4_end = c_begin + ((c_end - c_begin) & ~3LL);
    constexpr long long kStep = 4LL * kCntThreads;
    long long c = c_begin + 4LL * tid;
    for (; c + 3 * kStep < c4_end; c += 4 * kStep) {
      float4 v[4];
#pragma unroll
      for (int u = 0; u < 4; ++u) v[u] = ld_stream_f4(reinterpret_cast<const float4*>(drow + c + u * kStep));
#pragma unroll
      for (int u = 0; u < 4; ++u) {
        const long long cu = c + u * kStep;
        visit(v[u].x, cu); visit(v[u].y, cu + 1); visit(v[u].z, cu + 2); visit(v[u].w, cu + 3);
      }
    }
    for (; c < c4_end; c += kStep) {
      const float4 v = ld_stream_f4(reinterpret_cast<const float4*>(drow + c));
      visit(v.x, c); visit(v.y, c + 1); visit(v.z, c + 2); visit(v.w, c + 3);
    }
    for (c = c4_end + tid; c < c_end; c += kCntThreads) visit(drow[c], c);
  } else {
    for (long long c = c_begin + tid; c < c_end; c += kCntThreads) visit(drow[c], c);
  }

#pragma unroll
  for (int o = 16; o > 0; o >>= 1) {
    below += __shfl_xor_sync(0xffffffffu, below, o);
    tie_corr += __shfl_xor_sync(0xffffffffu, tie_corr, o);
  }
  if (lane == 0) {
    if (below) atomicAdd(&s_below, below);
    if (tie_corr) atomicAdd(&s_first_cnt, tie_corr);
  }
  __syncthreads();
  constexpr int kPer = kNB / kCntThreads;
  uint32_t local[kPer], sum = 0;
#pragma unroll
  for (int k = 0; k < kPer; ++k) {
    local[k] = hist[tid * kPer + k] & 0x7fffffffu;
    sum += local[k];
  }
  part[tid] = sum;
  __syncthreads();
  if (tid < 32) {
    uint32_t v[4], run = 0;
#pragma unroll
    for (int k = 0; k < 4; ++k) { v[k] = part[tid * 4 + k]; run += v[k]; }
    uint32_t incl = run;
#pragma unroll
    for (int o = 1; o < 32; o <<= 1) {
      const uint32_t t = __shfl_up_sync(0xffffffffu, incl, o);
      if (lane >= o) incl += t;
    }
    uint32_t excl = incl - run;
#pragma unroll
    for (int k = 0; k < 4; ++k) { part[tid * 4 + k] = excl; excl += v[k]; }
  }
  __syncthreads();
  {
    uint32_t run = part[tid];
#pragma unroll
    for (int k = 0; k < kPer; ++k) { hist[tid * kPer + k] = run; run += local[k]; }
  }
  __syncthreads();
  const uint32_t below_all = s_below;
  for (int p = tid; p < np; p += kCntThreads) {
    const unsigned b = ((unsigned)fkey(thr[p]) - (unsigned)key_min) >> shift;
    const int first = (int)(binfo[b] >> 16);
    uint32_t n = below_all + hist[b];
    for (int k = first; k <= p; ++k) n += exact[k];
    if (n) atomicAdd(&cnt_le[tpair[p]], n);
  }
  if (tid == 0 && s_first_cnt) atomicAdd(&cnt_first[q], s_first_cnt);
}

__global__ void __launch_bounds__(128) rank_finalize_kernel(long long nq, const int32_t* __restrict__ pair_off,
                                                            const int32_t* __restrict__ pair_g,
                                                            const uint8_t* __restrict__ pair_pos,
                                                            const float* __restrict__ pair_d,
                                                            const uint32_t* __restrict__ cnt_le,
                                                            const uint32_t* __restrict__ cnt_first,
                                                            double* __restrict__ ap, uint8_t* __restrict__ is_valid,
                                                            int32_t* __restrict__ first_rank,
                                                            int32_t* __restrict__ neg_before) {
  const int lane = threadIdx.x & 31;
  const long long q = (long long)blockIdx.x * 4 + (threadIdx.x >> 5);
  if (q >= nq) return;
  const int e0 = pair_off[q], e1 = pair_off[q + 1];
  double acc = 0.0;
  int np = 0;
  float dstar = FLT_MAX;
  int gstar = 0x7fffffff;
  uint32_t le_star = 0;
  for (int e = e0 + lane; e < e1; e += 32) {
    if (!pair_pos[e]) continue;
    const float d = pair_d[e];
    const int g = pair_g[e];
    int c_pos = 0, c_junk = 0;
    for (int f = e0; f < e1; ++f) {
      const bool le = pair_d[f] <= d;
      if (pair_pos[f]) c_pos += le; else c_junk += le;
    }
    const int n_valid = (int)cnt_le[e] - c_junk;
    acc += (double)c_pos / (double)n_valid;
    if (neg_before) neg_before[e] = n_valid - c_pos;
    ++np;
    if (d < dstar || (d == dstar && g < gstar)) { dstar = d; gstar = g; le_star = cnt_le[e]; }
  }
#pragma unroll
  for (int o = 16; o > 0; o >>= 1) {
    acc += __shfl_xor_sync(0xffffffffu, acc, o);
    np += __shfl_xor_sync(0xffffffffu, np, o);
    const float od = __shfl_xor_sync(0xffffffffu, dstar, o);
    const int og = __shfl_xor_sync(0xffffffffu, gstar, o);
    const uint32_t ol = __shfl_xor_sync(0xffffffffu, le_star, o);
    if (od < dstar || (od == dstar && og < gstar)) { dstar = od; gstar = og; le_star = ol; }
  }
  int jb = 0;
  if (np > 0) {
    for (int e = e0 + lane; e < e1; e += 32) {
      if (pair_pos[e]) continue;
      const float d = pair_d[e];
      jb += (d < dstar) || (d == dstar && pair_g[e] < gstar);
    }
#pragma unroll
    for (int o = 16; o > 0; o >>= 1) jb += __shfl_xor_sync(0xffffffffu, jb, o);
  }
  if (lane == 0) {
    ap[q] = np > 0 ? acc / (double)np : 0.0;
    is_valid[q] = np > 0 ? 1 : 0;
    first_rank[q] = np > 0 ? (int32_t)(le_star + cnt_first[q]) - jb : -1;
  }
}

template <bool TAGS>
__global__ void __launch_bounds__(kTopkThreads) topk_update_kernel(const float* __restrict__ dist, long long ldd,
                                                                    long long ncols, long long col0,
                                                                    const int32_t* __restrict__ excl_off,
                                                                    const int32_t* __restrict__ excl_g,
                                                                    const uint8_t* __restrict__ excl_keep,
                                                                    const long long* __restrict__ g_tags,
                                                                    const long long* __restrict__ q_tags,
                                                                    uint32_t* __restrict__ n_tag_excl,
                                                                    unsigned long long* __restrict__ topk_key, int k) {
  __shared__ unsigned long long cand[kCand];
  __shared__ int s_n;
  __shared__ unsigned long long s_bound;
  __shared__ uint32_t s_excl;
  const int q = blockIdx.x, tid = threadIdx.x;
  unsigned long long* state = topk_key + (long long)q * k;
  for (int i = tid; i < kCand; i += kTopkThreads) cand[i] = i < k ? state[i] : ~0ull;
  if (tid == 0) { s_n = k; s_bound = state[k - 1]; if (TAGS) s_excl = 0u; }
  __syncthreads();
  const float* drow = dist + (long long)q * ldd;
  const int x0 = excl_off ? excl_off[q] : 0, x1 = excl_off ? excl_off[q + 1] : 0;
  const long long qtag = TAGS ? q_tags[q] : 0;
  uint32_t n_tx = 0;
  const long long tile = 4LL * kTopkThreads;
  for (long long c0 = 0; c0 < ncols; c0 += tile) {
    const unsigned long long bound = s_bound;
#pragma unroll
    for (int u = 0; u < 4; ++u) {
      const long long c = c0 + (long long)u * kTopkThreads + tid;
      if (c < ncols) {
        const float d = ld_stream_f32(drow + c);
        const unsigned long long key = ((unsigned long long)__float_as_uint(d) << 32) | (unsigned long long)(uint32_t)(col0 + c);
        bool tag_out = false;
        if (TAGS && n_tag_excl) {
          tag_out = __ldg(g_tags + c) == qtag;
// ... 207 lines not shown
  __syncthreads();
  for (int i = tid; i < np; i += blockDim.x)
    if (se[i]) atomicAdd(&cnt_eq[e0 + i], se[i]);
}

__global__ void __launch_bounds__(128) rank_finalize_trapezoid_kernel(long long nq, const int32_t* __restrict__ pair_off,
                                                                      const int32_t* __restrict__ pair_g,
                                                                      const uint8_t* __restrict__ pair_pos,
                                                                      const float* __restrict__ pair_d,
                                                                      const uint32_t* __restrict__ cnt_le,
                                                                      const uint32_t* __restrict__ cnt_eq,
                                                                      double* __restrict__ ap) {
  const int lane = threadIdx.x & 31;
  const long long q = (long long)blockIdx.x * 4 + (threadIdx.x >> 5);
  if (q >= nq) return;
  const int e0 = pair_off[q], e1 = pair_off[q + 1];
  double acc = 0.0;
  int npos = 0;
  for (int e = e0 + lane; e < e1; e += 32) {
    if (!pair_pos[e]) continue;
    ++npos;
    const float d = pair_d[e];
    int tp = 0, tp_lt = 0, junk_le = 0, junk_eq = 0;
    bool rep = true;
    for (int f = e0; f < e1; ++f) {
      const float df = pair_d[f];
      if (pair_pos[f]) {
        tp += df <= d;
        tp_lt += df < d;
        rep &= !(df == d && f < e);
      } else {
        junk_le += df <= d;
        junk_eq += df == d;
      }
    }
    if (!rep) continue;
    const double n_le = (double)((int)cnt_le[e] - junk_le);
    const double n_lt = n_le - (double)((int)cnt_eq[e] - junk_eq);
    const double p_prev = n_lt > 0.0 ? (double)tp_lt / n_lt : 1.0;
    acc += (double)(tp - tp_lt) * ((double)tp / n_le + p_prev) * 0.5;
  }
#pragma unroll
  for (int o = 16; o > 0; o >>= 1) {
    acc += __shfl_xor_sync(0xffffffffu, acc, o);
    npos += __shfl_xor_sync(0xffffffffu, npos, o);
  }
  if (lane == 0) ap[q] = npos > 0 ? acc / (double)npos : 0.0;
  (void)pair_g;
}

}

using namespace pps;

namespace pps {
int rank_gather_ex(const float* dist, long long ldd, long long nq, long long ncols, long long col0, const int32_t* pair_q,
                   const int32_t* pair_g, long long n_pairs, float* pair_d, void* stream, const int32_t* n_dev) {
  if (nq < 0 || ncols < 0 || n_pairs < 0 || ldd < ncols) return PPS_ERR_INVALID_ARG;
  if (n_pairs == 0 || ncols == 0 || nq == 0) return PPS_OK;
  if (!dist || !pair_q || !pair_g || !pair_d) return PPS_ERR_INVALID_ARG;
  const long long blocks = (n_pairs + 255) / 256;
  if (blocks > 0x7fffffffLL) return PPS_ERR_UNSUPPORTED;
  rank_gather_kernel<<<(unsigned)blocks, 256, 0, static_cast<cudaStream_t>(stream)>>>(dist, ldd, ncols, col0, pair_q,
                                                                                      pair_g, n_pairs, pair_d, n_dev);
  PPS_LAUNCH_CHECK("rank_gather_kernel");
  return PPS_OK;
}
}

extern "C" int pps_rank_gather(const float* dist, long long ldd, long long nq, long long ncols, long long col0,
                               const int32_t* pair_q, const int32_t* pair_g, long long n_pairs, float* pair_d,
                               void* stream) {
  return rank_gather_ex(dist, ldd, nq, ncols, col0, pair_q, pair_g, n_pairs, pair_d, stream, nullptr);
}

static int rank_count_launch(const float* dist, long long ldd, long long nq, long long ncols, long long col0,
                             const int32_t* pair_off, const int32_t* pair_g, const uint8_t* pair_pos,
                             const float* pair_d, int max_pairs_per_query, uint32_t* cnt_le, uint32_t* cnt_first,
                             unsigned long long* topk_key, int k, int topk_filtered, void* stream) {
  const bool topk = topk_key != nullptr;
  const int maxp = ((max_pairs_per_query > 0 ? max_pairs_per_query : 1) + 3) & ~3;
  const size_t smem = (size_t)maxp * 24;
  if (smem > 150 * 1024) return PPS_ERR_UNSUPPORTED;
  const int sms = sm_count();
  long long splits = 1;
  if (!topk && nq < 4LL * sms) splits = (4LL * sms + nq - 1) / nq;
  long long seg = (ncols + splits - 1) / splits;
  seg = (seg + 1023) & ~1023LL;
  splits = (ncols + seg - 1) / seg;
  if (splits > 65535) return PPS_ERR_UNSUPPORTED;
  static thread_local int configured_dev = -1;
  int dev = 0;
  PPS_CUDA_TRY(cudaGetDevice(&dev));
  if (configured_dev != dev) {
    PPS_CUDA_TRY(cudaFuncSetAttribute(rank_count_kernel<false>, cudaFuncAttributeMaxDynamicSharedMemorySize, 150 * 1024));
    PPS_CUDA_TRY(cudaFuncSetAttribute(rank_count_kernel<true>, cudaFuncAttributeMaxDynamicSharedMemorySize, 150 * 1024));
    configured_dev = dev;
  }
  const dim3 grid((unsigned)nq, (unsigned)splits);
  cudaStream_t st = static_cast<cudaStream_t>(stream);
  if (topk)
    rank_count_kernel<true><<<grid, kCntThreads, smem, st>>>(dist, ldd, ncols, col0, seg, pair_off, pair_g, pair_pos,
                                                             pair_d, maxp, cnt_le, cnt_first, topk_key, k, topk_filtered);
  else
    rank_count_kernel<false><<<grid, kCntThreads, smem, st>>>(dist, ldd, ncols, col0, seg, pair_off, pair_g, pair_pos,
                                                              pair_d, maxp, cnt_le, cnt_first, nullptr, 0, 0);
  PPS_LAUNCH_CHECK("rank_count_kernel");
  return PPS_OK;
}

extern "C" int pps_rank_count(const float* dist, long long ldd, long long nq, long long ncols, long long col0,
                              const int32_t* pair_off, const int32_t* pair_g, const uint8_t* pair_pos,
                              const float* pair_d, int max_pairs_per_query, uint32_t* cnt_le, uint32_t* cnt_first,
                              void* stream) {
  if (nq < 0 || ncols < 0 || ldd < ncols || max_pairs_per_query < 0) return PPS_ERR_INVALID_ARG;
  if (nq == 0 || ncols == 0) return PPS_OK;
  if (!dist || !pair_off || !cnt_first) return PPS_ERR_INVALID_ARG;
  if (max_pairs_per_query == 0) return PPS_OK;
  if (!pair_g || !pair_pos || !pair_d || !cnt_le) return PPS_ERR_INVALID_ARG;
  if (nq > 0x7fffffffLL) return PPS_ERR_UNSUPPORTED;
  return rank_count_launch(dist, ldd, nq, ncols, col0, pair_off, pair_g, pair_pos, pair_d, max_pairs_per_query, cnt_le,
                           cnt_first, nullptr, 0, 0, stream);
}

extern "C" int pps_rank_sweep(const float* dist, long long ldd, long long nq, long long ncols, long long col0,
                              const int32_t* pair_off, const int32_t* pair_g, const uint8_t* pair_pos,
                              const float* pair_d, int max_pairs_per_query, uint32_t* cnt_le, uint32_t* cnt_first,
                              uint64_t* topk_key, int k, int topk_filtered, void* stream) {
  if (nq < 0 || ncols < 0 || ldd < ncols || max_pairs_per_query < 0 || k < 1 || k > PPS_TOPK_MAX) return PPS_ERR_INVALID_ARG;
  if (nq == 0 || ncols == 0) return PPS_OK;
  if (!dist || !pair_off || !cnt_first || !topk_key) return PPS_ERR_INVALID_ARG;
  if (max_pairs_per_query > 0 && (!pair_g || !pair_pos || !pair_d || !cnt_le)) return PPS_ERR_INVALID_ARG;
  if (nq > 0x7fffffffLL || col0 + ncols > 0xffffffffLL) return PPS_ERR_UNSUPPORTED;
  return rank_count_launch(dist, ldd, nq, ncols, col0, pair_off, pair_g, pair_pos, pair_d, max_pairs_per_query, cnt_le,
                           cnt_first, reinterpret_cast<unsigned long long*>(topk_key), k, topk_filtered, stream);
}

extern "C" int pps_rank_finalize(long long nq, const int32_t* pair_off, const int32_t* pair_g, const uint8_t* pair_pos,
                                 const float* pair_d, const uint32_t* cnt_le, const uint32_t* cnt_first, double* ap,
                                 uint8_t* is_valid, int32_t* first_rank, int32_t* neg_before, void* stream) {
  if (nq < 0) return PPS_ERR_INVALID_ARG;
  if (nq == 0) return PPS_OK;
  if (!pair_off || !cnt_first || !ap || !is_valid || !first_rank) return PPS_ERR_INVALID_ARG;
  const long long blocks = (nq + 3) / 4;
  if (blocks > 0x7fffffffLL) return PPS_ERR_UNSUPPORTED;
  rank_finalize_kernel<<<(unsigned)blocks, 128, 0, static_cast<cudaStream_t>(stream)>>>(
      nq, pair_off, pair_g, pair_pos, pair_d, cnt_le, cnt_first, ap, is_valid, first_rank, neg_before);
  PPS_LAUNCH_CHECK("rank_finalize_kernel");
  return PPS_OK;
}

extern "C" int pps_topk_init(uint64_t* topk_key, long long nq, int k, void* stream) {
  if (nq < 0 || k < 1 || k > PPS_TOPK_MAX) return PPS_ERR_INVALID_ARG;
  if (nq == 0) return PPS_OK;
  if (!topk_key) return PPS_ERR_INVALID_ARG;
  const long long n = nq * k, blocks = (n + 255) / 256;
  topk_fill_kernel<<<(unsigned)blocks, 256, 0, static_cast<cudaStream_t>(stream)>>>(
      reinterpret_cast<unsigned long long*>(topk_key), n);
  PPS_LAUNCH_CHECK("topk_fill_kernel");
  return PPS_OK;
}

extern "C" int pps_topk_update(const float* dist, long long ldd, long long nq, long long ncols, long long col0,
                               const int32_t* excl_off, const int32_t* excl_g, const uint8_t* excl_keep,
                               uint64_t* topk_key, int k, void* stream) {
  if (nq < 0 || ncols < 0 || ldd < ncols || k < 1 || k > PPS_TOPK_MAX) return PPS_ERR_INVALID_ARG;
  if (nq == 0 || ncols == 0) return PPS_OK;
  if (!dist || !topk_key) return PPS_ERR_INVALID_ARG;
  if (excl_off && !excl_g) return PPS_ERR_INVALID_ARG;
  if (nq > 0x7fffffffLL || col0 + ncols > 0xffffffffLL) return PPS_ERR_UNSUPPORTED;
  topk_update_kernel<false><<<(unsigned)nq, kTopkThreads, 0, static_cast<cudaStream_t>(stream)>>>(
      dist, ldd, ncols, col0, excl_off, excl_g, excl_keep, nullptr, nullptr, nullptr,
      reinterpret_cast<unsigned long long*>(topk_key), k);
  PPS_LAUNCH_CHECK("topk_update_kernel");
  return PPS_OK;
}

extern "C" int pps_topk_update_excl(const float* dist, long long ldd, long long nq, long long ncols, long long col0,
                                    const int64_t* g_tags, const int64_t* q_tags, uint64_t* topk_key, int k,
                                    uint32_t* n_excluded, void* stream) {
  if (nq < 0 || ncols < 0 || ldd < ncols || k < 1 || k > PPS_TOPK_MAX) return PPS_ERR_INVALID_ARG;
  if (nq == 0) return PPS_OK;
  if (!topk_key || !q_tags || (ncols > 0 && (!dist || !g_tags))) return PPS_ERR_INVALID_ARG;
  if (nq > 0x7fffffffLL || col0 + ncols > 0xffffffffLL) return PPS_ERR_UNSUPPORTED;
  if (ncols == 0) {
    if (n_excluded) PPS_CUDA_TRY(cudaMemsetAsync(n_excluded, 0, (size_t)nq * sizeof(uint32_t), static_cast<cudaStream_t>(stream)));
    return PPS_OK;
  }
  topk_update_kernel<true><<<(unsigned)nq, kTopkThreads, 0, static_cast<cudaStream_t>(stream)>>>(
      dist, ldd, ncols, col0, nullptr, nullptr, nullptr, reinterpret_cast<const long long*>(g_tags),
      reinterpret_cast<const long long*>(q_tags), n_excluded, reinterpret_cast<unsigned long long*>(topk_key), k);
  PPS_LAUNCH_CHECK("topk_update_kernel<excl>");
  return PPS_OK;
}

extern "C" int pps_topk_unpack(const uint64_t* topk_key, long long nq, int k, float* out_dist, int32_t* out_index,
                               void* stream) {
  if (nq < 0 || k < 1 || k > PPS_TOPK_MAX) return PPS_ERR_INVALID_ARG;
  if (nq == 0) return PPS_OK;
  if (!topk_key) return PPS_ERR_INVALID_ARG;
  const long long n = nq * k, blocks = (n + 255) / 256;
  topk_unpack_kernel<<<(unsigned)blocks, 256, 0, static_cast<cudaStream_t>(stream)>>>(
      reinterpret_cast<const unsigned long long*>(topk_key), n, out_dist, out_index);
  PPS_LAUNCH_CHECK("topk_unpack_kernel");
  return PPS_OK;
}

extern "C" long long pps_rank_tab_elems(long long nq, int p_cap) {
  if (nq < 0 || p_cap < 8 || p_cap > 64 || (p_cap & 7)) return PPS_ERR_INVALID_ARG;
  const long long rows_pad = (nq + 255) / 256 * 256;
  return rows_pad * p_cap;
}

extern "C" int pps_rank_tab_prep(long long nq, const int32_t* pair_off, const int32_t* pair_g, const uint8_t* pair_pos,
                                 const float* pair_d, int p_cap, float* thr_tab, int32_t* tpair_tab, uint32_t* cnt_tab,
                                 float* dstar, int32_t* gstar, int32_t* overflow, void* stream) {
  if (nq < 0 || p_cap < 8 || p_cap > 64 || (p_cap & 7)) return PPS_ERR_INVALID_ARG;
  if (nq == 0) return PPS_OK;
  if (!pair_off || !thr_tab || !tpair_tab || !cnt_tab || !dstar || !gstar || !overflow) return PPS_ERR_INVALID_ARG;
  const long long rows_pad = (nq + 255) / 256 * 256;
  cudaStream_t st = static_cast<cudaStream_t>(stream);
  PPS_CUDA_TRY(cudaMemsetAsync(overflow, 0, 4, st));
  rank_tab_prep_kernel<<<(unsigned)(rows_pad / 4), 128, 0, st>>>(nq, rows_pad, pair_off, pair_g, pair_pos, pair_d, p_cap,
                                                                thr_tab, tpair_tab, cnt_tab, dstar, gstar, overflow);
  PPS_LAUNCH_CHECK("rank_tab_prep_kernel");
  return PPS_OK;
}

extern "C" int pps_rank_tab_finish(long long nq, int p_cap, const int32_t* tpair_tab, const uint32_t* cnt_tab,
                                   uint32_t* cnt_le, void* stream) {
  if (nq < 0 || p_cap < 8 || p_cap > 64 || (p_cap & 7)) return PPS_ERR_INVALID_ARG;
  if (nq == 0) return PPS_OK;
// ... 80 lines not shown
```

pps_b200/csrc/split_prep.cu:

```cuda
#include "common.cuh"

namespace pps {

constexpr int kSplitWarps = 8;

template <int PLANES, bool F16IN>
__global__ void __launch_bounds__(32 * kSplitWarps) split_rows_kernel(const void* __restrict__ feats, long long row_begin,
                                                                       long long row_end, long long rows, int dim,
                                                                       long long ld, int kpad,
                                                                       void* __restrict__ out_planes,
                                                                       float* __restrict__ out_sqnorm,
                                                                       const int32_t* __restrict__ row_index,
                                                                       long long index_base) {
  const int lane = threadIdx.x & 31;
  const long long row = row_begin + (long long)blockIdx.x * kSplitWarps + (threadIdx.x >> 5);
  if (row >= row_end) return;
  const long long srow = row_index ? (long long)row_index[row] - index_base : row;
  double acc = 0.0;
  const long long plane_stride = rows * (long long)kpad;
  if constexpr (F16IN) {
    const __half* src = reinterpret_cast<const __half*>(feats) + srow * ld;
    __half* dst = out_planes ? reinterpret_cast<__half*>(out_planes) + row * (long long)kpad : nullptr;
    const bool vec8 = ((dim & 7) == 0) && ((ld & 7) == 0) && ((reinterpret_cast<uintptr_t>(feats) & 15u) == 0);
    if (vec8) {
      for (int k = lane * 8; k < dim; k += 256) {
        const uint4 u = *reinterpret_cast<const uint4*>(src + k);
        const __half2* h2 = reinterpret_cast<const __half2*>(&u);
#pragma unroll
        for (int e = 0; e < 4; ++e) {
          const float2 f = __half22float2(h2[e]);
          acc += (double)(f.x * f.x) + (double)(f.y * f.y);
        }
        if (dst) *reinterpret_cast<uint4*>(dst + k) = u;
      }
      if (dst)
        for (int k = dim + lane; k < kpad; k += 32) dst[k] = __float2half(0.f);
    } else {
      for (int k = lane; k < kpad; k += 32) {
        const __half h = k < dim ? src[k] : __float2half(0.f);
        const float v = __half2float(h);
        acc += (double)v * (double)v;
        if (dst) dst[k] = h;
      }
    }
  } else {
    const float* src = reinterpret_cast<const float*>(feats) + srow * ld;
    __nv_bfloat16* dst = reinterpret_cast<__nv_bfloat16*>(out_planes);
    const bool vec = ((ld & 3) == 0) && ((reinterpret_cast<uintptr_t>(feats) & 15u) == 0);
    int kfast = lane * 4;
    if (vec) {
      for (; kfast + 3 * 128 + 3 < dim; kfast += 4 * 128) {
        float4 t[4];
#pragma unroll
        for (int u = 0; u < 4; ++u) t[u] = ld_stream_f4(reinterpret_cast<const float4*>(src + kfast + u * 128));
#pragma unroll
        for (int u = 0; u < 4; ++u) {
          const int k = kfast + u * 128;
          const float v[4] = {t[u].x, t[u].y, t[u].z, t[u].w};
          __nv_bfloat16 p[3][4];
#pragma unroll
          for (int e = 0; e < 4; ++e) {
            acc += (double)v[e] * (double)v[e];
            float r = v[e];
#pragma unroll
            for (int pl = 0; pl < PLANES; ++pl) {
              p[pl][e] = __float2bfloat16_rn(r);
              r -= __bfloat162float(p[pl][e]);
            }
          }
          if (dst) {
#pragma unroll
            for (int pl = 0; pl < PLANES; ++pl) {
              uint2 w;
              w.x = (uint32_t)__bfloat16_as_ushort(p[pl][0]) | ((uint32_t)__bfloat16_as_ushort(p[pl][1]) << 16);
              w.y = (uint32_t)__bfloat16_as_ushort(p[pl][2]) | ((uint32_t)__bfloat16_as_ushort(p[pl][3]) << 16);
              *reinterpret_cast<uint2*>(dst + pl * plane_stride + row * (long long)kpad + k) = w;
            }
          }
        }
      }
    }
    for (int k = kfast; k < kpad; k += 128) {
      float v[4];
      if (vec && k + 3 < dim) {
        const float4 t = ld_stream_f4(reinterpret_cast<const float4*>(src + k));
        v[0] = t.x; v[1] = t.y; v[2] = t.z; v[3] = t.w;
      } else {
#pragma unroll
        for (int e = 0; e < 4; ++e) v[e] = (k + e < dim) ? src[k + e] : 0.f;
      }
      __nv_bfloat16 p[3][4];
#pragma unroll
      for (int e = 0; e < 4; ++e) {
        acc += (double)v[e] * (double)v[e];
        float r = v[e];
#pragma unroll
        for (int pl = 0; pl < PLANES; ++pl) {
          p[pl][e] = __float2bfloat16_rn(r);
          r -= __bfloat162float(p[pl][e]);
        }
      }
      if (dst) {
#pragma unroll
        for (int pl = 0; pl < PLANES; ++pl) {
          uint2 w;
          w.x = (uint32_t)__bfloat16_as_ushort(p[pl][0]) | ((uint32_t)__bfloat16_as_ushort(p[pl][1]) << 16);
          w.y = (uint32_t)__bfloat16_as_ushort(p[pl][2]) | ((uint32_t)__bfloat16_as_ushort(p[pl][3]) << 16);
          *reinterpret_cast<uint2*>(dst + pl * plane_stride + row * (long long)kpad + k) = w;
        }
      }
    }
  }
#pragma unroll
  for (int o = 16; o > 0; o >>= 1) acc += __shfl_xor_sync(0xffffffffu, acc, o);
  if (lane == 0 && out_sqnorm) out_sqnorm[row] = (float)acc;
}

template <int kF16Cache4>
__global__ void __launch_bounds__(32 * kSplitWarps) split_rows_f16s_kernel(const float* __restrict__ feats, long long row_begin,
                                                                            long long row_end, long long rows, int dim,
                                                                            long long ld, int kpad,
                                                                            __half* __restrict__ out_planes,
                                                                            float* __restrict__ out_sqnorm,
                                                                            const int32_t* __restrict__ row_index,
                                                                            long long index_base) {
  const int lane = threadIdx.x & 31;
  const long long row = row_begin + (long long)blockIdx.x * kSplitWarps + (threadIdx.x >> 5);
  if (row >= row_end) return;
  const long long srow = row_index ? (long long)row_index[row] - index_base : row;
  const float* src = feats + srow * ld;
  const bool vec = ((ld & 3) == 0) && ((reinterpret_cast<uintptr_t>(feats) & 15u) == 0);
  auto load4 = [&](int k, bool stream) -> float4 {
    if (vec && k + 3 < dim)
      return stream ? ld_stream_f4(reinterpret_cast<const float4*>(src + k)) : *reinterpret_cast<const float4*>(src + k);
    float4 t;
    t.x = k < dim ? src[k] : 0.f;
    t.y = k + 1 < dim ? src[k + 1] : 0.f;
    t.z = k + 2 < dim ? src[k + 2] : 0.f;
    t.w = k + 3 < dim ? src[k + 3] : 0.f;
    return t;
  };
  double acc = 0.0;
  float mx = 0.f;
  auto note = [&](const float4& t) {
    acc += (double)t.x * (double)t.x + (double)t.y * (double)t.y + (double)t.z * (double)t.z + (double)t.w * (double)t.w;
    mx = fmaxf(mx, fmaxf(fmaxf(fabsf(t.x), fabsf(t.y)), fmaxf(fabsf(t.z), fabsf(t.w))));
  };
  float4 cache[kF16Cache4 > 0 ? kF16Cache4 : 1];
#pragma unroll
  for (int u = 0; u < kF16Cache4; ++u) {
    const int k = lane * 4 + u * 128;
    cache[u] = k < kpad ? load4(k, true) : make_float4(0.f, 0.f, 0.f, 0.f);
    note(cache[u]);
  }
  {
    int k = lane * 4 + kF16Cache4 * 128;
    for (; k + 3 * 128 < kpad; k += 4 * 128) {
      float4 t[4];
#pragma unroll
      for (int u = 0; u < 4; ++u) t[u] = load4(k + u * 128, false);
#pragma unroll
      for (int u = 0; u < 4; ++u) note(t[u]);
    }
    for (; k < kpad; k += 128) note(load4(k, false));
  }
#pragma unroll
  for (int o = 16; o > 0; o >>= 1) {
    acc += __shfl_xor_sync(0xffffffffu, acc, o);
    mx = fmaxf(mx, __shfl_xor_sync(0xffffffffu, mx, o));
  }
  int e = 0;
  if (mx > 0.f && mx <= 3.0e38f) {
    int ex;
    frexpf(mx, &ex);
    e = 15 - ex;
    e = e > 100 ? 100 : (e < -100 ? -100 : e);
  }
  const float s = ldexpf(1.f, e), inv = ldexpf(1.f, -e);
  const long long plane_stride = rows * (long long)kpad;
  __half* dst = out_planes + row * (long long)kpad;
  auto emit = [&](int k, const float4& t) {
    const float2 a = make_float2(t.x * s, t.y * s), b = make_float2(t.z * s, t.w * s);
    const __half2 ha = __float22half2_rn(a), hb = __float22half2_rn(b);
    const float2 fa = __half22float2(ha), fb = __half22float2(hb);
    const __half2 la = __float22half2_rn(make_float2(a.x - fa.x, a.y - fa.y));
    const __half2 lb = __float22half2_rn(make_float2(b.x - fb.x, b.y - fb.y));
    uint2 w0, w1;
    w0.x = *reinterpret_cast<const uint32_t*>(&ha);
    w0.y = *reinterpret_cast<const uint32_t*>(&hb);
    w1.x = *reinterpret_cast<const uint32_t*>(&la);
    w1.y = *reinterpret_cast<const uint32_t*>(&lb);
    *reinterpret_cast<uint2*>(dst + k) = w0;
    *reinterpret_cast<uint2*>(dst + plane_stride + k) = w1;
  };
#pragma unroll
  for (int u = 0; u < kF16Cache4; ++u) {
    const int k = lane * 4 + u * 128;
    if (k < kpad) emit(k, cache[u]);
  }
  {
    int k = lane * 4 + kF16Cache4 * 128;
    for (; k + 3 * 128 < kpad; k += 4 * 128) {
      float4 t[4];
#pragma unroll
      for (int u = 0; u < 4; ++u) t[u] = load4(k + u * 128, false);
#pragma unroll
      for (int u = 0; u < 4; ++u) emit(k + u * 128, t[u]);
    }
    for (; k < kpad; k += 128) emit(k, load4(k, false));
  }
  if (lane == 0 && out_sqnorm) {
    out_sqnorm[row] = (float)acc;
    out_sqnorm[rows + row] = inv;
  }
}

__global__ void __launch_bounds__(256) l2_normalize_rows_kernel(const float* __restrict__ x, int dim, long long ld,
                                                                float* __restrict__ out, long long ldo) {
  __shared__ float part[8];
  const float* src = x + (long long)blockIdx.x * ld;
  float* dst = out + (long long)blockIdx.x * ldo;
  const bool vec = ((dim & 3) == 0) && ((ld & 3) == 0) && ((ldo & 3) == 0) &&
                   (((reinterpret_cast<uintptr_t>(x) | reinterpret_cast<uintptr_t>(out)) & 15u) == 0);
  float acc = 0.f;
  if (vec) {
    for (int k = threadIdx.x * 4; k < dim; k += 1024) {
      const float4 t = *reinterpret_cast<const float4*>(src + k);
      acc = fmaf(t.x, t.x, acc); acc = fmaf(t.y, t.y, acc); acc = fmaf(t.z, t.z, acc); acc = fmaf(t.w, t.w, acc);
    }
  } else {
    for (int k = threadIdx.x; k < dim; k += 256) acc = fmaf(src[k], src[k], acc);
  }
#pragma unroll
  for (int o = 16; o > 0; o >>= 1) acc += __shfl_xor_sync(0xffffffffu, acc, o);
  if ((threadIdx.x & 31) == 0) part[threadIdx.x >> 5] = acc;
  __syncthreads();
  float tot = 0.f;
#pragma unroll
  for (int w = 0; w < 8; ++w) tot += part[w];
  const float inv = 1.0f / fmaxf(sqrtf(tot), 1e-12f);
  if (vec) {
    for (int k = threadIdx.x * 4; k < dim; k += 1024) {
      float4 t = *reinterpret_cast<const float4*>(src + k);
      t.x *= inv; t.y *= inv; t.z *= inv; t.w *= inv;
      *reinterpret_cast<float4*>(dst + k) = t;
    }
  } else {
    for (int k = threadIdx.x; k < dim; k += 256) dst[k] = src[k] * inv;
  }
}

__global__ void __launch_bounds__(256) group_mean_rows_kernel(const float* __restrict__ feats, long long ld, int dim,
                                                              const int32_t* __restrict__ group_off,
                                                              const int32_t* __restrict__ row_idx, float* __restrict__ out,
                                                              long long ldo) {
  const int gidx = blockIdx.x;
  const int e0 = group_off[gidx], e1 = group_off[gidx + 1];
  const float cnt = (float)(e1 - e0);
  for (int c = threadIdx.x; c < dim; c += blockDim.x) {
    float acc = 0.f;
    for (int e = e0; e < e1; ++e) acc = __fadd_rn(acc, feats[(long long)row_idx[e] * ld + c]);
    out[(long long)gidx * ldo + c] = e1 > e0 ? __fdiv_rn(acc, cnt) : 0.f;
  }
}

}

using namespace pps;

extern "C" int pps_kpad(int dim) { return dim <= 0 ? 0 : ((dim + 63) / 64) * 64; }

extern "C" long long pps_split_bytes(long long rows, int dim, int planes) {
  if (planes & PPS_SPLIT_F16_SCALED) planes = 2;
  if (rows < 0 || dim <= 0 || planes < 1 || planes > 3) return PPS_ERR_INVALID_ARG;
  return rows * (long long)pps_kpad(dim) * 2 * planes;
}

static int split_dispatch(const void* feats, int dtype, long long row0, long long nrows, long long rows, int dim,
                          long long ld, int planes, void* out_planes, float* out_sqnorm, void* stream,
                          const int32_t* row_index = nullptr, long long index_base = 0) {
  if (rows < 0 || dim <= 0 || ld < dim || row0 < 0 || nrows < 0 || row0 + nrows > rows) return PPS_ERR_INVALID_ARG;
  if (nrows == 0) return PPS_OK;
  if (!feats) return PPS_ERR_INVALID_ARG;
  if (out_planes && (reinterpret_cast<uintptr_t>(out_planes) & 15u)) return PPS_ERR_ALIGN;
  const int kpad = pps_kpad(dim);
  const long long blocks = (nrows + kSplitWarps - 1) / kSplitWarps;
  if (blocks > 0x7fffffffLL) return PPS_ERR_UNSUPPORTED;
  cudaStream_t st = static_cast<cudaStream_t>(stream);
  const dim3 grid((unsigned)blocks), block(32 * kSplitWarps);
  if (dtype == PPS_DTYPE_F16) {
    if (planes != 1) return PPS_ERR_INVALID_ARG;
    split_rows_kernel<1, true><<<grid, block, 0, st>>>(feats, row0, row0 + nrows, rows, dim, ld, kpad, out_planes, out_sqnorm, row_index, index_base);
  } else if (dtype == PPS_DTYPE_F32 && (planes & PPS_SPLIT_F16_SCALED)) {
    if ((planes & ~PPS_SPLIT_F16_SCALED) != 2 || !out_planes || !out_sqnorm) return PPS_ERR_INVALID_ARG;
    split_rows_f16s_kernel<0><<<grid, block, 0, st>>>(static_cast<const float*>(feats), row0, row0 + nrows, rows, dim, ld, kpad,
                                                      static_cast<__half*>(out_planes), out_sqnorm, row_index, index_base);
  } else if (dtype == PPS_DTYPE_F32) {
    switch (planes) {
      case 1: split_rows_kernel<1, false><<<grid, block, 0, st>>>(feats, row0, row0 + nrows, rows, dim, ld, kpad, out_planes, out_sqnorm, row_index, index_base); break;
      case 2: split_rows_kernel<2, false><<<grid, block, 0, st>>>(feats, row0, row0 + nrows, rows, dim, ld, kpad, out_planes, out_sqnorm, row_index, index_base); break;
      case 3: split_rows_kernel<3, false><<<grid, block, 0, st>>>(feats, row0, row0 + nrows, rows, dim, ld, kpad, out_planes, out_sqnorm, row_index, index_base); break;
      default: return PPS_ERR_INVALID_ARG;
    }
  } else {
    return PPS_ERR_INVALID_ARG;
  }
  PPS_LAUNCH_CHECK("split_rows_kernel");
  return PPS_OK;
}

extern "C" int pps_split_rows(const void* feats, int dtype, long long rows, int dim, long long ld, int planes,
                              void* out_planes, float* out_sqnorm, void* stream) {
  if (!out_planes && rows > 0) return PPS_ERR_INVALID_ARG;
  return split_dispatch(feats, dtype, 0, rows, rows, dim, ld, planes, out_planes, out_sqnorm, stream);
}

extern "C" int pps_split_rows_slab(const void* feats, int dtype, long long row0, long long nrows, long long total_rows,
                                   int dim, long long ld, int planes, void* out_planes, float* out_sqnorm,
                                   void* stream) {
  if (!out_planes && nrows > 0) return PPS_ERR_INVALID_ARG;
  return split_dispatch(feats, dtype, row0, nrows, total_rows, dim, ld, planes, out_planes, out_sqnorm, stream);
}

extern "C" int pps_row_sqnorm(const void* feats, int dtype, long long rows, int dim, long long ld, float* out_sqnorm,
                              void* stream) {
  if (!out_sqnorm && rows > 0) return PPS_ERR_INVALID_ARG;
  return split_dispatch(feats, dtype, 0, rows, rows, dim, ld, 1, nullptr, out_sqnorm, stream);
}

extern "C" int pps_l2_normalize_rows(const float* x, long long rows, int dim, long long ld, float* out, long long ldo,
                                     void* stream) {
  if (rows < 0 || dim <= 0 || ld < dim || ldo < dim) return PPS_ERR_INVALID_ARG;
  if (rows == 0) return PPS_OK;
  if (!x || !out) return PPS_ERR_INVALID_ARG;
  if (rows > 0x7fffffffLL) return PPS_ERR_UNSUPPORTED;
  l2_normalize_rows_kernel<<<(unsigned)rows, 256, 0, static_cast<cudaStream_t>(stream)>>>(x, dim, ld, out, ldo);
  PPS_LAUNCH_CHECK("l2_normalize_rows_kernel");
  return PPS_OK;
}

extern "C" int pps_split_rows_gather(const void* feats, int dtype, const int32_t* row_index, long long index_base,
                                     long long rows, int dim, long long ld, int planes, void* out_planes,
                                     float* out_sqnorm, void* stream) {
  if ((!out_planes || !row_index) && rows > 0) return PPS_ERR_INVALID_ARG;
  return split_dispatch(feats, dtype, 0, rows, rows, dim, ld, planes, out_planes, out_sqnorm, stream, row_index,
                        index_base);
}

extern "C" int pps_group_mean_rows(const float* feats, long long ld, int dim, const int32_t* group_off,
                                   const int32_t* row_idx, long long n_groups, float* out, long long ldo, void* stream) {
  if (n_groups < 0 || dim <= 0 || ld < dim || ldo < dim) return PPS_ERR_INVALID_ARG;
  if (n_groups == 0) return PPS_OK;
  if (!feats || !group_off || !row_idx || !out) return PPS_ERR_INVALID_ARG;
  if (n_groups > 0x7fffffffLL) return PPS_ERR_UNSUPPORTED;
  group_mean_rows_kernel<<<(unsigned)n_groups, 256, 0, static_cast<cudaStream_t>(stream)>>>(feats, ld, dim, group_off, row_idx,
                                                                                          out, ldo);
  PPS_LAUNCH_CHECK("group_mean_rows_kernel");
  return PPS_OK;
}
```

Before: 74.78 billion.

## Merge split launches, fuse pair count with offsets and clamp, trim memsets

Query and gallery row splitting now runs in one kernel launch over two row sets. The pair count sweep accumulates per-query totals atomically, so the separate rowsum kernel is gone, and offset clamping moves into the offsets kernel, which drops the clamp kernel. Several memsets are skipped when a single device or no top-k is used, and the side stream gets high priority. Together these cut launch count and serialization on the short critical path, at the cost of atomics in the count sweep and an extra wait on the pairs event before distance when world is 1.

```diff
diff --git a/pps_b200/build.py b/pps_b200/build.py
--- a/pps_b200/build.py
+++ b/pps_b200/build.py
@@ -80,8 +80,9 @@
 
 
 def build_test_hooks(force: bool = False) -> str:
+    build()
     src = os.path.join(CSRC, "test_hooks.cu")
-    deps = [src] + [h for h in HEADERS if os.path.exists(h)]
+    deps = [src, LIB_PATH] + [h for h in HEADERS if os.path.exists(h)]
     if (not force and os.path.exists(TEST_HOOKS_PATH)
             and all(os.path.getmtime(d) <= os.path.getmtime(TEST_HOOKS_PATH) for d in deps)):
         return TEST_HOOKS_PATH
@@ -90,7 +91,8 @@
         raise RuntimeError("nvcc not found: cannot build the test hooks")
     os.makedirs(OUT_DIR, exist_ok=True)
     tmp = TEST_HOOKS_PATH + ".tmp.%d" % os.getpid()
-    proc = subprocess.run([nvcc] + NVCC_FLAGS + ["-shared", "-o", tmp, "test_hooks.cu"], cwd=CSRC, stdout=subprocess.PIPE,
+    link = ["-L" + OUT_DIR, "-lpps_b200", "-Xlinker", "-rpath,$ORIGIN"]
+    proc = subprocess.run([nvcc] + NVCC_FLAGS + ["-shared", "-o", tmp, "test_hooks.cu"] + link, cwd=CSRC, stdout=subprocess.PIPE,
                           stderr=subprocess.STDOUT, text=True)
     if proc.returncode != 0:
         raise RuntimeError("nvcc failed on test_hooks.cu:\n%s" % proc.stdout)
diff --git a/pps_b200/csrc/c_api.cu b/pps_b200/csrc/c_api.cu
--- a/pps_b200/csrc/c_api.cu
+++ b/pps_b200/csrc/c_api.cu
@@ -132,7 +132,11 @@
   c->device = device;
   cudaError_t e = cudaStreamCreateWithFlags(&c->copy_s, cudaStreamNonBlocking);
   if (e == cudaSuccess) e = cudaStreamCreateWithFlags(&c->comp_s, cudaStreamNonBlocking);
-  if (e == cudaSuccess) e = cudaStreamCreateWithFlags(&c->side_s, cudaStreamNonBlocking);
+  if (e == cudaSuccess) {
+    int lo = 0, hi = 0;
+    e = cudaDeviceGetStreamPriorityRange(&lo, &hi);
+    if (e == cudaSuccess) e = cudaStreamCreateWithPriority(&c->side_s, cudaStreamNonBlocking, hi);
+  }
   if (e == cudaSuccess) e = cudaEventCreateWithFlags(&c->ev_in, cudaEventDisableTiming);
   if (e == cudaSuccess) e = cudaEventCreateWithFlags(&c->ev_pairs, cudaEventDisableTiming);
   for (int i = 0; i < kMaxSlabs && e == cudaSuccess; ++i) e = cudaEventCreateWithFlags(&c->ev_slab[i], cudaEventDisableTiming);
@@ -425,8 +429,8 @@
   PPS_TRY(pairs_local_count(c, cs));
   if (d_local_cnt) *d_local_cnt = c->local_cnt;
   mark(c, 1, cs);
-  PPS_TRY(pps_split_rows(d_q, PPS_DTYPE_F32, e.nq, e.dim, e.dim, e.split_planes, c->qs.p, c->qn.as<float>(), cs));
-  PPS_TRY(pps_split_rows(d_g, PPS_DTYPE_F32, e.ng, e.dim, e.dim, e.split_planes, c->gs.p, c->gn.as<float>(), cs));
+  PPS_TRY(split_rows_pair(d_q, e.nq, c->qs.p, c->qn.as<float>(), d_g, e.ng, c->gs.p, c->gn.as<float>(), PPS_DTYPE_F32, e.dim,
+                          e.split_planes, cs));
   mark(c, 2, cs);
   PPS_TRY(pps_dist_tc(c->qs.p, c->qn.as<float>(), e.nq, e.planes, 0, c->gs.p, c->gn.as<float>(), e.ng, e.planes, 0,
                       e.dim, e.precision, world > 1 ? PPS_DIST_RESERVE_SM_PAIR : 0, c->dist.as<float>(), e.ldd, cs));
diff --git a/pps_b200/csrc/common.cuh b/pps_b200/csrc/common.cuh
--- a/pps_b200/csrc/common.cuh
+++ b/pps_b200/csrc/common.cuh
@@ -27,6 +27,13 @@
   } while (0)
 
 int sm_count();
+
+struct FinalizeFlags {
+  const uint32_t* src = nullptr;
+  uint32_t* dst = nullptr;
+  const int32_t* tot = nullptr;
+  int32_t cap_pairs = 0, cap_maxp = 0, cap_cand = -1, cap_rows = -1;
+};
 
 #ifdef __CUDACC__
 
diff --git a/pps_b200/csrc/ctx.cuh b/pps_b200/csrc/ctx.cuh
--- a/pps_b200/csrc/ctx.cuh
+++ b/pps_b200/csrc/ctx.cuh
@@ -54,7 +54,7 @@
 };
 
 int pairs_count_device_ex(const int64_t* query_ids, long long nq, const int64_t* gallery_ids, long long ng_cap, void* workspace,
-                          int32_t* pair_off, int32_t* totals, void* stream, const int32_t* ng_dev);
+                          int32_t* pair_off, int32_t* totals, void* stream, const int32_t* ng_dev, long long cap);
 int pairs_fill_device_ex(const int64_t* query_ids, const int64_t* query_cams, long long nq, const int64_t* gallery_ids,
                          const int64_t* gallery_cams, long long ng_cap, const void* workspace, int32_t* pair_q, int32_t* pair_g,
                          uint8_t* pair_pos, float* zero_f32, uint32_t* zero_u32, uint32_t* zero_per_query, long long capacity,
@@ -67,6 +67,11 @@
                           long long rows_cap);
 int rank_gather_ex(const float* dist, long long ldd, long long nq, long long ncols, long long col0, const int32_t* pair_q,
                    const int32_t* pair_g, long long n_pairs, float* pair_d, void* stream, const int32_t* n_dev);
+int rank_finalize_ex(long long nq, const int32_t* pair_off, const int32_t* pair_g, const uint8_t* pair_pos, const float* pair_d,
+                     const uint32_t* cnt_le, const uint32_t* cnt_first, double* ap, uint8_t* is_valid, int32_t* first_rank,
+                     int32_t* neg_before, const FinalizeFlags& flags, void* stream);
+int split_rows_pair(const void* feats_a, long long rows_a, void* planes_a, float* norms_a, const void* feats_b,
+                    long long rows_b, void* planes_b, float* norms_b, int dtype, int dim, int planes, cudaStream_t st);
 
 constexpr int kPassMaxBlocks = 4096;
 constexpr int kPassTimedLaunches = 256;
diff --git a/pps_b200/csrc/pairs.cu b/pps_b200/csrc/pairs.cu
--- a/pps_b200/csrc/pairs.cu
+++ b/pps_b200/csrc/pairs.cu
@@ -16,7 +16,8 @@
                    int32_t* __restrict__ pair_g, uint8_t* __restrict__ pair_pos, int32_t* __restrict__ pair_pos32,
                    float* __restrict__ zero_f32, uint32_t* __restrict__ zero_u32,
                    uint32_t* __restrict__ zero_per_query, long long capacity,
-                   const int32_t* __restrict__ ng_dev ) {
+                   const int32_t* __restrict__ ng_dev ,
+                   int32_t* __restrict__ q_total ) {
   if (ng_dev) ng = min(ng, (long long)*ng_dev);
   const int lane = threadIdx.x & 31, warp = threadIdx.x >> 5;
   const int q0 = blockIdx.x * kPairQPerCta + warp * kPairQPerWarp;
@@ -85,7 +86,10 @@
   if (!FILL && lane == 0) {
 #pragma unroll
     for (int u = 0; u < kPairQPerWarp; ++u)
-      if (live[u]) seg_cnt[(long long)(q0 + u) * nseg + s] = acc[u];
+      if (live[u]) {
+        seg_cnt[(long long)(q0 + u) * nseg + s] = acc[u];
+        if (q_total && acc[u]) atomicAdd(&q_total[q0 + u], acc[u]);
+      }
   }
 }
 
@@ -100,7 +104,8 @@
 
 __global__ void __launch_bounds__(1024) pairs_offsets_kernel(const int32_t* __restrict__ cnt_all, int world, int rank,
                                                              int nq, int32_t* __restrict__ pair_off,
-                                                             int32_t* __restrict__ my_base, int32_t* __restrict__ totals) {
+                                                             int32_t* __restrict__ my_base, int32_t* __restrict__ totals,
+                                                             int32_t cap) {
   __shared__ int warp_sum[32];
   __shared__ int carry_s;
   __shared__ int max_s;
@@ -140,7 +145,7 @@
     const int carry = carry_s;
     if (q < nq) {
       const int off = carry + (warp ? warp_sum[warp - 1] : 0) + incl - sum;
-      pair_off[q] = off;
+      pair_off[q] = cap >= 0 ? min(off, cap) : off;
       my_base[q] = off + before;
     }
     __syncthreads();
@@ -151,7 +156,7 @@
   for (int o = 16; o > 0; o >>= 1) mx = max(mx, __shfl_xor_sync(0xffffffffu, mx, o));
   if (lane == 0) atomicMax(&max_s, mx);
   __syncthreads();
-  if (tid == 0) { pair_off[nq] = carry_s; totals[0] = carry_s; totals[1] = max_s; }
+  if (tid == 0) { pair_off[nq] = cap >= 0 ? min(carry_s, cap) : carry_s; totals[0] = carry_s; totals[1] = max_s; }
 }
 
 __global__ void pairs_unpack_pos_kernel(const int32_t* __restrict__ pos32, long long n, uint8_t* __restrict__ pos8) {
@@ -433,7 +438,7 @@
   const dim3 grid((unsigned)((nq + kPairQPerCta - 1) / kPairQPerCta), (unsigned)nseg);
   pairs_sweep_kernel<false><<<grid, 32 * kPairWarps, 0, st>>>(query_ids, nullptr, (int)nq, gallery_ids, nullptr, ng, seg,
                                                               nseg, seg_cnt, nullptr, 0, nullptr, nullptr, nullptr,
-                                                              nullptr, nullptr, nullptr, nullptr, 0, ng_dev);
+                                                              nullptr, nullptr, nullptr, nullptr, 0, ng_dev, nullptr);
   PPS_LAUNCH_CHECK("pairs_sweep_kernel<count>");
   pairs_rowsum_kernel<<<(unsigned)((nq + 255) / 256), 256, 0, st>>>(seg_cnt, (int)nq, nseg, lc);
   PPS_LAUNCH_CHECK("pairs_rowsum_kernel");
@@ -454,7 +459,7 @@
   ws_ints(nq, ng_local, &nseg);
   int32_t* my_base = static_cast<int32_t*>(workspace) + (nq > 0 ? nq : 1) * ((long long)nseg + 1);
   pairs_offsets_kernel<<<1, 1024, 0, static_cast<cudaStream_t>(stream)>>>(cnt_all, world, rank, (int)nq, pair_off, my_base,
-                                                                          totals);
+                                                                          totals, -1);
   PPS_LAUNCH_CHECK("pairs_offsets_kernel");
   return PPS_OK;
 }
@@ -484,7 +489,7 @@
   pairs_sweep_kernel<true><<<grid, 32 * kPairWarps, 0, st>>>(query_ids, query_cams, (int)nq, gallery_ids, gallery_cams, ng,
                                                              seg, nseg, seg_cnt, my_base, gallery_offset, pair_q, pair_g,
                                                              pair_pos, pair_pos32, zero_f32, zero_u32, zero_per_query,
-                                                             capacity, ng_dev);
+                                                             capacity, ng_dev, nullptr);
   PPS_LAUNCH_CHECK("pairs_sweep_kernel<fill>");
   return PPS_OK;
 }
@@ -520,12 +525,28 @@
 
 namespace pps {
 int pairs_count_device_ex(const int64_t* query_ids, long long nq, const int64_t* gallery_ids, long long ng_cap, void* workspace,
-                          int32_t* pair_off, int32_t* totals, void* stream, const int32_t* ng_dev) {
-  if (!pair_off || !totals) return PPS_ERR_INVALID_ARG;
-  int32_t* lc = nullptr;
-  int rc = pairs_local_count_ex(query_ids, nq, gallery_ids, ng_cap, workspace, &lc, stream, ng_dev);
-  if (rc != PPS_OK) return rc;
-  return pps_pairs_offsets(lc, 1, 0, nq, ng_cap, workspace, pair_off, totals, stream);
+                          int32_t* pair_off, int32_t* totals, void* stream, const int32_t* ng_dev, long long cap) {
+  if (!pair_off || !totals || !workspace) return PPS_ERR_INVALID_ARG;
+  if (nq < 0 || ng_cap < 0 || nq > 0x7fffffffLL || ng_cap > 0x7fffffffLL || cap > 0x7fffffffLL) return PPS_ERR_INVALID_ARG;
+  if (nq > 0 && ng_cap > 0 && (!query_ids || !gallery_ids)) return PPS_ERR_INVALID_ARG;
+  cudaStream_t st = static_cast<cudaStream_t>(stream);
+  long long seg; int nseg;
+  pair_segments(ng_cap, &seg, &nseg);
+  if ((long long)nq * nseg > 0x7fffffffLL) return PPS_ERR_UNSUPPORTED;
+  int32_t* seg_cnt = static_cast<int32_t*>(workspace);
+  int32_t* lc = seg_cnt + (nq > 0 ? nq : 1) * (long long)nseg;
+  int32_t* my_base = lc + (nq > 0 ? nq : 1);
+  if (nq > 0) PPS_CUDA_TRY(cudaMemsetAsync(ng_cap > 0 ? lc : seg_cnt, 0, (size_t)nq * (ng_cap > 0 ? 1 : nseg + 1) * 4, st));
+  if (nq > 0 && ng_cap > 0) {
+    const dim3 grid((unsigned)((nq + kPairQPerCta - 1) / kPairQPerCta), (unsigned)nseg);
+    pairs_sweep_kernel<false><<<grid, 32 * kPairWarps, 0, st>>>(query_ids, nullptr, (int)nq, gallery_ids, nullptr, ng_cap, seg,
+                                                                nseg, seg_cnt, nullptr, 0, nullptr, nullptr, nullptr,
+                                                                nullptr, nullptr, nullptr, nullptr, 0, ng_dev, lc);
+    PPS_LAUNCH_CHECK("pairs_sweep_kernel<count>");
+  }
+  pairs_offsets_kernel<<<1, 1024, 0, st>>>(lc, 1, 0, (int)nq, pair_off, my_base, totals, (int32_t)cap);
+  PPS_LAUNCH_CHECK("pairs_offsets_kernel");
+  return PPS_OK;
 }
 int pairs_fill_device_ex(const int64_t* query_ids, const int64_t* query_cams, long long nq, const int64_t* gallery_ids,
                          const int64_t* gallery_cams, long long ng_cap, const void* workspace, int32_t* pair_q, int32_t* pair_g,
diff --git a/pps_b200/csrc/pass.cu b/pps_b200/csrc/pass.cu
--- a/pps_b200/csrc/pass.cu
+++ b/pps_b200/csrc/pass.cu
@@ -51,15 +51,6 @@
 
 __global__ void pass_or_flag_kernel(const int32_t* __restrict__ src, uint32_t* __restrict__ dst) {
   if (threadIdx.x == 0 && blockIdx.x == 0 && *src) *dst = 1u;
-}
-
-__global__ void pass_copy_flags_kernel(const uint32_t* __restrict__ src, uint32_t* __restrict__ dst) {
-  if (threadIdx.x < 2 && blockIdx.x == 0) dst[threadIdx.x] = src[threadIdx.x];
-}
-
-__global__ void pass_clamp_offsets_kernel(int32_t* __restrict__ pair_off, long long n, int32_t cap) {
-  const long long i = (long long)blockIdx.x * blockDim.x + threadIdx.x;
-  if (i < n && pair_off[i] > cap) pair_off[i] = cap;
 }
 
 __global__ void pass_check_bounds_kernel(const int32_t* __restrict__ tot, int32_t cap_pairs, int32_t cap_maxp, int32_t cap_cand,
@@ -258,13 +249,13 @@
     }
   }
 
-  {
-    TimedLaunch t(c, cs, 1);
-    PPS_TRY(pps_split_rows(d_q, dtype, nq, dim, dim, p.split_planes, p.qs.p, p.qn.as<float>(), cs));
-  }
   const void* gp0 = nullptr;
   long long slab = 0;
   if (slabbed) {
+    {
+      TimedLaunch t(c, cs, 1);
+      PPS_TRY(pps_split_rows(d_q, dtype, nq, dim, dim, p.split_planes, p.qs.p, p.qn.as<float>(), cs));
+    }
     unsigned char* dg = static_cast<unsigned char*>(const_cast<void*>(d_g));
     const unsigned char* hg = static_cast<const unsigned char*>(h_g);
     slab = ((ng_local + 7) / 8 + 255) & ~255LL;
@@ -277,8 +268,17 @@
       PPS_CUDA_TRY(cudaMemcpyAsync(dg + off, hg + off, (size_t)nr * dim * esz_in, cudaMemcpyHostToDevice, c->copy_s));
       PPS_CUDA_TRY(cudaEventRecord(c->ev_slab[si], c->copy_s));
     }
-  } else if (p.n_blocks > 0) {
-    PPS_TRY(split_block(c, 0, p.blk_row0[0], p.blk_rows[0], cs, &gp0));
+  } else {
+    const long long rows0 = p.n_blocks > 0 ? p.blk_rows[0] : 0;
+    const unsigned char* src0 = static_cast<const unsigned char*>(d_g);
+    if (p.n_blocks > 0) {
+      src0 += (size_t)p.blk_row0[0] * dim * esz_in;
+      if (p.g_from_host) PPS_CUDA_TRY(cudaStreamWaitEvent(cs, c->ev_slab[0], 0));
+      gp0 = p.g_inplace ? static_cast<const void*>(src0) : p.gs.p;
+    }
+    TimedLaunch t(c, cs, 1);
+    PPS_TRY(split_rows_pair(d_q, nq, p.qs.p, p.qn.as<float>(), src0, rows0, p.g_inplace ? nullptr : p.gs.p, p.gn.as<float>(),
+                            dtype, dim, p.split_planes, cs));
   }
 
   PassState::Hints& hn = p.hints;
@@ -306,13 +306,14 @@
     dn_cand = d_tot + 2;
   }
   PPS_TRY(p.pair_ws.ensure((size_t)std::max<long long>(pps_pairs_workspace_bytes(nq, sweep_rows), 16)));
-  PPS_TRY(pairs_count_device_ex(d_qid, nq, sweep_gid, sweep_rows, p.pair_ws.p, p.pair_off.as<int32_t>(), d_tot, ss, dn_cand));
   if (spec) {
     p.n_pairs = hn.n_pairs > 0 ? (hn.n_pairs + hn.n_pairs / 8 + 1023) / 1024 * 1024 : 0;
     p.max_pairs = hn.max_pairs > 0 ? (hn.max_pairs + 8 + 15) / 16 * 16 : 0;
-    pass_clamp_offsets_kernel<<<(unsigned)((nq + 1 + 255) / 256), 256, 0, ss>>>(p.pair_off.as<int32_t>(), nq + 1, (int32_t)p.n_pairs);
-    PPS_LAUNCH_CHECK("pass_clamp_offsets_kernel");
-  } else {
+  }
+  PPS_CUDA_TRY(cudaMemsetAsync(d_tot + 3, 0, 4, ss));
+  PPS_TRY(pairs_count_device_ex(d_qid, nq, sweep_gid, sweep_rows, p.pair_ws.p, p.pair_off.as<int32_t>(), d_tot, ss, dn_cand,
+                                spec ? p.n_pairs : -1));
+  if (!spec) {
     PPS_CUDA_TRY(cudaMemcpyAsync(h_tot, d_tot, 8, cudaMemcpyDeviceToHost, ss));
     PPS_CUDA_TRY(cudaEventRecord(c->ev_totals, ss));
     {
@@ -331,14 +332,14 @@
     p.p_cap = std::max(8, (need + 7) / 8 * 8);
   }
   PPS_TRY(p.small.ensure(16));
-  PPS_CUDA_TRY(cudaMemsetAsync(p.small.p, 0, 16, ss));
+  if (p.epi_topk) PPS_CUDA_TRY(cudaMemsetAsync(p.small.p, 0, 16, ss));
   PPS_TRY(p.pair_q.ensure(np1 * 4));
   PPS_TRY(p.pair_g.ensure(np1 * 4));
   PPS_TRY(p.pair_pos.ensure(np1));
   PPS_TRY(p.pair_d.ensure(np1 * 4));
   p.packed_bytes = ((size_t)nq * topk * 8 + p.counter_words() * 4 + 15) & ~(size_t)15;
   PPS_TRY(p.packed.ensure(p.packed_bytes));
-  if (spec) {
+  if (spec && world > 1) {
     PPS_CUDA_TRY(cudaMemsetAsync(p.pair_d.p, 0, np1 * 4, ss));
     PPS_CUDA_TRY(cudaMemsetAsync(p.cnt_first(), 0, p.counter_words() * 4, ss));
     PPS_CUDA_TRY(cudaMemsetAsync(p.pair_q.p, 0xFF, np1 * 4, ss));
@@ -363,7 +364,6 @@
   }
   p.n_rows = 0;
   p.cap_rows = 0;
-  PPS_CUDA_TRY(cudaMemsetAsync(d_tot + 3, 0, 4, ss));
   if (p.n_blocks > 1 && p.n_pairs > 0) {
     PPS_TRY(p.gp_ws.ensure((size_t)pps_pairs_compact_workspace_bytes(nq)));
     if (spec) p.cap_rows = hn.n_rows > 0 ? std::min<long long>((hn.n_rows + 255) / 256 * 256, std::max<long long>(p.ngl, 1)) : 0;
@@ -414,6 +414,7 @@
                           precision, world > 1 ? PPS_DIST_RESERVE_SM_PAIR : 0, p.dist.as<float>() + r0, p.ldd, cs));
     }
   } else if (p.n_blocks > 0) {
+    if (world == 1) PPS_CUDA_TRY(cudaStreamWaitEvent(cs, c->ev_pairs, 0));
     PPS_TRY(distance_block(c, gp0, p.blk_rows[0], p.offset + p.blk_row0[0], false, cs));
   }
   PPS_CUDA_TRY(cudaStreamWaitEvent(cs, c->ev_pairs, 0));
@@ -536,7 +537,7 @@
     pass_or_flag_kernel<<<1, 32, 0, cs>>>(p.small.as<int32_t>() + 1, p.flags_dev() + 1);
     PPS_LAUNCH_CHECK("pass_or_flag_kernel");
   }
-  if (p.speculative) {
+  if (p.speculative && p.world > 1) {
     pass_check_bounds_kernel<<<1, 32, 0, cs>>>(p.totals.as<int32_t>(), (int32_t)p.n_pairs, (int32_t)p.max_pairs,
                                                p.prefilter ? (int32_t)p.cap_cand : -1,
                                                p.n_blocks > 1 ? (int32_t)p.cap_rows : -1, p.flags_dev() + 1);
@@ -575,12 +576,20 @@
   }
   {
     TimedLaunch t(c, cs, 5);
-    PPS_TRY(pps_rank_finalize(nq, p.pair_off.as<int32_t>(), p.pair_g.as<int32_t>(), p.pair_pos.as<uint8_t>(),
-                              p.pair_d.as<float>(), p.cnt_le(), p.cnt_first(), p.ap.as<double>(),
-                              p.ap.as<uint8_t>() + p.res_valid_off,
-                              reinterpret_cast<int32_t*>(p.ap.as<unsigned char>() + p.res_first_off), nullptr, cs));
-    pass_copy_flags_kernel<<<1, 32, 0, cs>>>(p.flags_dev(), reinterpret_cast<uint32_t*>(p.ap.as<unsigned char>() + p.res_flags_off));
-    PPS_LAUNCH_CHECK("pass_copy_flags_kernel");
+    FinalizeFlags fl;
+    fl.src = p.flags_dev();
+    fl.dst = reinterpret_cast<uint32_t*>(p.ap.as<unsigned char>() + p.res_flags_off);
+    if (p.speculative && p.world == 1) {
+      fl.tot = p.totals.as<int32_t>();
+      fl.cap_pairs = (int32_t)p.n_pairs;
+      fl.cap_maxp = (int32_t)p.max_pairs;
+      fl.cap_cand = p.prefilter ? (int32_t)p.cap_cand : -1;
+      fl.cap_rows = p.n_blocks > 1 ? (int32_t)p.cap_rows : -1;
+    }
+    PPS_TRY(rank_finalize_ex(nq, p.pair_off.as<int32_t>(), p.pair_g.as<int32_t>(), p.pair_pos.as<uint8_t>(),
+                             p.pair_d.as<float>(), p.cnt_le(), p.cnt_first(), p.ap.as<double>(),
+                             p.ap.as<uint8_t>() + p.res_valid_off,
+                             reinterpret_cast<int32_t*>(p.ap.as<unsigned char>() + p.res_first_off), nullptr, fl, cs));
     if (topk > 0) {
       PPS_TRY(p.tki.ensure((size_t)nq * topk * 4));
       PPS_TRY(p.tkd.ensure((size_t)nq * topk * 4));
diff --git a/pps_b200/csrc/rank.cu b/pps_b200/csrc/rank.cu
--- a/pps_b200/csrc/rank.cu
+++ b/pps_b200/csrc/rank.cu
@@ -361,9 +361,17 @@
                                                             const uint32_t* __restrict__ cnt_first,
                                                             double* __restrict__ ap, uint8_t* __restrict__ is_valid,
                                                             int32_t* __restrict__ first_rank,
-                                                            int32_t* __restrict__ neg_before) {
+                                                            int32_t* __restrict__ neg_before, const FinalizeFlags fl) {
   const int lane = threadIdx.x & 31;
   const long long q = (long long)blockIdx.x * 4 + (threadIdx.x >> 5);
+  if (fl.dst && blockIdx.x == 0 && threadIdx.x == 0) {
+    uint32_t f1 = fl.src[1];
+    if (fl.tot && (fl.tot[0] > fl.cap_pairs || fl.tot[1] > fl.cap_maxp || (fl.cap_cand >= 0 && fl.tot[2] > fl.cap_cand) ||
+                   (fl.cap_rows >= 0 && fl.tot[3] > fl.cap_rows)))
+      f1 = 1u;
+    fl.dst[0] = fl.src[0];
+    fl.dst[1] = f1;
+  }
   if (q >= nq) return;
   const int e0 = pair_off[q], e1 = pair_off[q + 1];
   double acc = 0.0;
@@ -737,21 +745,40 @@
   const int maxp = ((max_pairs_per_query > 0 ? max_pairs_per_query : 1) + 3) & ~3;
   const size_t smem = (size_t)maxp * 24;
   if (smem > 150 * 1024) return PPS_ERR_UNSUPPORTED;
-  const int sms = sm_count();
-  long long splits = 1;
-  if (!topk && nq < 4LL * sms) splits = (4LL * sms + nq - 1) / nq;
-  long long seg = (ncols + splits - 1) / splits;
-  seg = (seg + 1023) & ~1023LL;
-  splits = (ncols + seg - 1) / seg;
-  if (splits > 65535) return PPS_ERR_UNSUPPORTED;
   static thread_local int configured_dev = -1;
+  static thread_local size_t occ_smem = 0;
+  static thread_local int occ = 0;
   int dev = 0;
   PPS_CUDA_TRY(cudaGetDevice(&dev));
   if (configured_dev != dev) {
     PPS_CUDA_TRY(cudaFuncSetAttribute(rank_count_kernel<false>, cudaFuncAttributeMaxDynamicSharedMemorySize, 150 * 1024));
     PPS_CUDA_TRY(cudaFuncSetAttribute(rank_count_kernel<true>, cudaFuncAttributeMaxDynamicSharedMemorySize, 150 * 1024));
     configured_dev = dev;
-  }
+    occ = 0;
+  }
+  const int sms = sm_count();
+  long long splits = 1;
+  if (!topk && nq < 4LL * sms) {
+    splits = (4LL * sms + nq - 1) / nq;
+  } else if (!topk) {
+    if (occ == 0 || occ_smem != smem) {
+      PPS_CUDA_TRY(cudaOccupancyMaxActiveBlocksPerMultiprocessor(&occ, rank_count_kernel<false>, kCntThreads, smem));
+      if (occ < 1) occ = 1;
+      occ_smem = smem;
+    }
+    const long long wave = (long long)sms * occ;
+    double best = 0.0;
+    for (long long s = 1; s <= 8; ++s) {
+      const long long ctas = nq * s, waves = (ctas + wave - 1) / wave;
+      const double fill = (double)ctas / (double)(waves * wave);
+      if (fill > best) { best = fill; splits = s; }
+      if (fill >= 0.9) break;
+    }
+  }
+  long long seg = (ncols + splits - 1) / splits;
+  seg = (seg + 1023) & ~1023LL;
+  splits = (ncols + seg - 1) / seg;
+  if (splits > 65535) return PPS_ERR_UNSUPPORTED;
   const dim3 grid((unsigned)nq, (unsigned)splits);
   cudaStream_t st = static_cast<cudaStream_t>(stream);
   if (topk)
@@ -791,18 +818,27 @@
                            cnt_first, reinterpret_cast<unsigned long long*>(topk_key), k, topk_filtered, stream);
 }
 
+namespace pps {
+int rank_finalize_ex(long long nq, const int32_t* pair_off, const int32_t* pair_g, const uint8_t* pair_pos, const float* pair_d,
+                     const uint32_t* cnt_le, const uint32_t* cnt_first, double* ap, uint8_t* is_valid, int32_t* first_rank,
+                     int32_t* neg_before, const FinalizeFlags& flags, void* stream) {
+  if (nq < 0) return PPS_ERR_INVALID_ARG;
+  if (nq == 0) return PPS_OK;
+  if (!pair_off || !cnt_first || !ap || !is_valid || !first_rank || (flags.dst && !flags.src)) return PPS_ERR_INVALID_ARG;
+  const long long blocks = (nq + 3) / 4;
+  if (blocks > 0x7fffffffLL) return PPS_ERR_UNSUPPORTED;
+  rank_finalize_kernel<<<(unsigned)blocks, 128, 0, static_cast<cudaStream_t>(stream)>>>(
+      nq, pair_off, pair_g, pair_pos, pair_d, cnt_le, cnt_first, ap, is_valid, first_rank, neg_before, flags);
+  PPS_LAUNCH_CHECK("rank_finalize_kernel");
+  return PPS_OK;
+}
+}
+
 extern "C" int pps_rank_finalize(long long nq, const int32_t* pair_off, const int32_t* pair_g, const uint8_t* pair_pos,
                                  const float* pair_d, const uint32_t* cnt_le, const uint32_t* cnt_first, double* ap,
                                  uint8_t* is_valid, int32_t* first_rank, int32_t* neg_before, void* stream) {
-  if (nq < 0) return PPS_ERR_INVALID_ARG;
-  if (nq == 0) return PPS_OK;
-  if (!pair_off || !cnt_first || !ap || !is_valid || !first_rank) return PPS_ERR_INVALID_ARG;
-  const long long blocks = (nq + 3) / 4;
-  if (blocks > 0x7fffffffLL) return PPS_ERR_UNSUPPORTED;
-  rank_finalize_kernel<<<(unsigned)blocks, 128, 0, static_cast<cudaStream_t>(stream)>>>(
-      nq, pair_off, pair_g, pair_pos, pair_d, cnt_le, cnt_first, ap, is_valid, first_rank, neg_before);
-  PPS_LAUNCH_CHECK("rank_finalize_kernel");
-  return PPS_OK;
+  return rank_finalize_ex(nq, pair_off, pair_g, pair_pos, pair_d, cnt_le, cnt_first, ap, is_valid, first_rank, neg_before,
+                          FinalizeFlags{}, stream);
 }
 
 extern "C" int pps_topk_init(uint64_t* topk_key, long long nq, int k, void* stream) {
diff --git a/pps_b200/csrc/split_prep.cu b/pps_b200/csrc/split_prep.cu
--- a/pps_b200/csrc/split_prep.cu
+++ b/pps_b200/csrc/split_prep.cu
@@ -1,21 +1,28 @@
-#include "common.cuh"
+#include "ctx.cuh"
 
 namespace pps {
 
 constexpr int kSplitWarps = 8;
 
+struct SplitSet {
+  const void* feats;
+  long long row_begin, row_end, rows, ld;
+  void* out_planes;
+  float* out_sqnorm;
+  const int32_t* row_index;
+  long long index_base;
+};
+
 template <int PLANES, bool F16IN>
-__global__ void __launch_bounds__(32 * kSplitWarps) split_rows_kernel(const void* __restrict__ feats, long long row_begin,
-                                                                       long long row_end, long long rows, int dim,
-                                                                       long long ld, int kpad,
-                                                                       void* __restrict__ out_planes,
-                                                                       float* __restrict__ out_sqnorm,
-                                                                       const int32_t* __restrict__ row_index,
-                                                                       long long index_base) {
+__device__ __forceinline__ void split_rows_body(const SplitSet& S, long long blk, int dim, int kpad) {
+  const void* __restrict__ feats = S.feats;
+  const long long rows = S.rows, ld = S.ld;
+  void* __restrict__ out_planes = S.out_planes;
+  float* __restrict__ out_sqnorm = S.out_sqnorm;
   const int lane = threadIdx.x & 31;
-  const long long row = row_begin + (long long)blockIdx.x * kSplitWarps + (threadIdx.x >> 5);
-  if (row >= row_end) return;
-  const long long srow = row_index ? (long long)row_index[row] - index_base : row;
+  const long long row = S.row_begin + blk * kSplitWarps + (threadIdx.x >> 5);
+  if (row >= S.row_end) return;
+  const long long srow = S.row_index ? (long long)S.row_index[row] - S.index_base : row;
   double acc = 0.0;
   const long long plane_stride = rows * (long long)kpad;
   if constexpr (F16IN) {
@@ -116,18 +123,23 @@
   if (lane == 0 && out_sqnorm) out_sqnorm[row] = (float)acc;
 }
 
+template <int PLANES, bool F16IN>
+__global__ void __launch_bounds__(32 * kSplitWarps) split_rows_kernel(const SplitSet a, const SplitSet b, long long a_blocks,
+                                                                       int dim, int kpad) {
+  if ((long long)blockIdx.x < a_blocks) split_rows_body<PLANES, F16IN>(a, blockIdx.x, dim, kpad);
+  else split_rows_body<PLANES, F16IN>(b, (long long)blockIdx.x - a_blocks, dim, kpad);
+}
+
 template <int kF16Cache4>
-__global__ void __launch_bounds__(32 * kSplitWarps) split_rows_f16s_kernel(const float* __restrict__ feats, long long row_begin,
-                                                                            long long row_end, long long rows, int dim,
-                                                                            long long ld, int kpad,
-                                                                            __half* __restrict__ out_planes,
-                                                                            float* __restrict__ out_sqnorm,
-                                                                            const int32_t* __restrict__ row_index,
-                                                                            long long index_base) {
+__device__ __forceinline__ void split_rows_f16s_body(const SplitSet& S, long long blk, int dim, int kpad) {
+  const float* __restrict__ feats = static_cast<const float*>(S.feats);
+  const long long rows = S.rows, ld = S.ld;
+  __half* __restrict__ out_planes = static_cast<__half*>(S.out_planes);
+  float* __restrict__ out_sqnorm = S.out_sqnorm;
   const int lane = threadIdx.x & 31;
-  const long long row = row_begin + (long long)blockIdx.x * kSplitWarps + (threadIdx.x >> 5);
-  if (row >= row_end) return;
-  const long long srow = row_index ? (long long)row_index[row] - index_base : row;
+  const long long row = S.row_begin + blk * kSplitWarps + (threadIdx.x >> 5);
+  if (row >= S.row_end) return;
+  const long long srow = S.row_index ? (long long)S.row_index[row] - S.index_base : row;
   const float* src = feats + srow * ld;
   const bool vec = ((ld & 3) == 0) && ((reinterpret_cast<uintptr_t>(feats) & 15u) == 0);
   auto load4 = [&](int k, bool stream) -> float4 {
@@ -215,6 +227,13 @@
   }
 }
 
+template <int kF16Cache4>
+__global__ void __launch_bounds__(32 * kSplitWarps) split_rows_f16s_kernel(const SplitSet a, const SplitSet b,
+                                                                            long long a_blocks, int dim, int kpad) {
+  if ((long long)blockIdx.x < a_blocks) split_rows_f16s_body<kF16Cache4>(a, blockIdx.x, dim, kpad);
+  else split_rows_f16s_body<kF16Cache4>(b, (long long)blockIdx.x - a_blocks, dim, kpad);
+}
+
 __global__ void __launch_bounds__(256) l2_normalize_rows_kernel(const float* __restrict__ x, int dim, long long ld,
                                                                 float* __restrict__ out, long long ldo) {
   __shared__ float part[8];
@@ -276,30 +295,38 @@
   return rows * (long long)pps_kpad(dim) * 2 * planes;
 }
 
-static int split_dispatch(const void* feats, int dtype, long long row0, long long nrows, long long rows, int dim,
-                          long long ld, int planes, void* out_planes, float* out_sqnorm, void* stream,
-                          const int32_t* row_index = nullptr, long long index_base = 0) {
-  if (rows < 0 || dim <= 0 || ld < dim || row0 < 0 || nrows < 0 || row0 + nrows > rows) return PPS_ERR_INVALID_ARG;
-  if (nrows == 0) return PPS_OK;
-  if (!feats) return PPS_ERR_INVALID_ARG;
-  if (out_planes && (reinterpret_cast<uintptr_t>(out_planes) & 15u)) return PPS_ERR_ALIGN;
+static int check_set(const SplitSet& S, int dim) {
+  if (S.rows < 0 || dim <= 0 || S.ld < dim || S.row_begin < 0 || S.row_end < S.row_begin || S.row_end > S.rows)
+    return PPS_ERR_INVALID_ARG;
+  if (S.row_end == S.row_begin) return PPS_OK;
+  if (!S.feats) return PPS_ERR_INVALID_ARG;
+  if (S.out_planes && (reinterpret_cast<uintptr_t>(S.out_planes) & 15u)) return PPS_ERR_ALIGN;
+  return PPS_OK;
+}
+
+static int split_launch(int dtype, int dim, int planes, const SplitSet& a, const SplitSet& b, void* stream) {
+  PPS_TRY(check_set(a, dim));
+  PPS_TRY(check_set(b, dim));
+  const long long a_blocks = (a.row_end - a.row_begin + kSplitWarps - 1) / kSplitWarps;
+  const long long blocks = a_blocks + (b.row_end - b.row_begin + kSplitWarps - 1) / kSplitWarps;
+  if (blocks == 0) return PPS_OK;
+  if (blocks > 0x7fffffffLL) return PPS_ERR_UNSUPPORTED;
   const int kpad = pps_kpad(dim);
-  const long long blocks = (nrows + kSplitWarps - 1) / kSplitWarps;
-  if (blocks > 0x7fffffffLL) return PPS_ERR_UNSUPPORTED;
   cudaStream_t st = static_cast<cudaStream_t>(stream);
   const dim3 grid((unsigned)blocks), block(32 * kSplitWarps);
   if (dtype == PPS_DTYPE_F16) {
     if (planes != 1) return PPS_ERR_INVALID_ARG;
-    split_rows_kernel<1, true><<<grid, block, 0, st>>>(feats, row0, row0 + nrows, rows, dim, ld, kpad, out_planes, out_sqnorm, row_index, index_base);
+    split_rows_kernel<1, true><<<grid, block, 0, st>>>(a, b, a_blocks, dim, kpad);
   } else if (dtype == PPS_DTYPE_F32 && (planes & PPS_SPLIT_F16_SCALED)) {
-    if ((planes & ~PPS_SPLIT_F16_SCALED) != 2 || !out_planes || !out_sqnorm) return PPS_ERR_INVALID_ARG;
-    split_rows_f16s_kernel<0><<<grid, block, 0, st>>>(static_cast<const float*>(feats), row0, row0 + nrows, rows, dim, ld, kpad,
-                                                      static_cast<__half*>(out_planes), out_sqnorm, row_index, index_base);
+    if ((planes & ~PPS_SPLIT_F16_SCALED) != 2) return PPS_ERR_INVALID_ARG;
+    for (const SplitSet* S : {&a, &b})
+      if (S->row_end > S->row_begin && (!S->out_planes || !S->out_sqnorm)) return PPS_ERR_INVALID_ARG;
+    split_rows_f16s_kernel<0><<<grid, block, 0, st>>>(a, b, a_blocks, dim, kpad);
   } else if (dtype == PPS_DTYPE_F32) {
     switch (planes) {
-      case 1: split_rows_kernel<1, false><<<grid, block, 0, st>>>(feats, row0, row0 + nrows, rows, dim, ld, kpad, out_planes, out_sqnorm, row_index, index_base); break;
-      case 2: split_rows_kernel<2, false><<<grid, block, 0, st>>>(feats, row0, row0 + nrows, rows, dim, ld, kpad, out_planes, out_sqnorm, row_index, index_base); break;
-      case 3: split_rows_kernel<3, false><<<grid, block, 0, st>>>(feats, row0, row0 + nrows, rows, dim, ld, kpad, out_planes, out_sqnorm, row_index, index_base); break;
+      case 1: split_rows_kernel<1, false><<<grid, block, 0, st>>>(a, b, a_blocks, dim, kpad); break;
+      case 2: split_rows_kernel<2, false><<<grid, block, 0, st>>>(a, b, a_blocks, dim, kpad); break;
+      case 3: split_rows_kernel<3, false><<<grid, block, 0, st>>>(a, b, a_blocks, dim, kpad); break;
       default: return PPS_ERR_INVALID_ARG;
     }
   } else {
@@ -307,6 +334,25 @@
   }
   PPS_LAUNCH_CHECK("split_rows_kernel");
   return PPS_OK;
+}
+
+static int split_dispatch(const void* feats, int dtype, long long row0, long long nrows, long long rows, int dim,
+                          long long ld, int planes, void* out_planes, float* out_sqnorm, void* stream,
+                          const int32_t* row_index = nullptr, long long index_base = 0) {
+  if (nrows < 0) return PPS_ERR_INVALID_ARG;
+  const SplitSet a{feats, row0, row0 + nrows, rows, ld, out_planes, out_sqnorm, row_index, index_base};
+  const SplitSet none{nullptr, 0, 0, 0, ld, nullptr, nullptr, nullptr, 0};
+  return split_launch(dtype, dim, planes, a, none, stream);
+}
+
+namespace pps {
+int split_rows_pair(const void* feats_a, long long rows_a, void* planes_a, float* norms_a, const void* feats_b,
+                    long long rows_b, void* planes_b, float* norms_b, int dtype, int dim, int planes, cudaStream_t st) {
+  if (rows_a < 0 || rows_b < 0 || (rows_a > 0 && !planes_a)) return PPS_ERR_INVALID_ARG;
+  const SplitSet a{feats_a, 0, rows_a, rows_a, dim, planes_a, norms_a, nullptr, 0};
+  const SplitSet b{feats_b, 0, rows_b, rows_b, dim, planes_b, norms_b, nullptr, 0};
+  return split_launch(dtype, dim, planes, a, b, st);
+}
 }
 
 extern "C" int pps_split_rows(const void* feats, int dtype, long long rows, int dim, long long ld, int planes,
```

Measured after the change: 76.05 billion (median of 6 runs). 1.02x the previous value.
